# larskaislaniemi/PyLamp

Hardware: AMD Instinct MI355X
Metric: stokes_heat_mic_cell_updates_per_s (higher is better)
Workload: dtype f64

## Files before the change

include/pylamp_hip.h:

```cpp
#ifndef PYLAMP_HIP_H
#define PYLAMP_HIP_H

#include <stddef.h>
#include <stdint.h>

#ifdef __cplusplus
extern "C" {
#endif

typedef struct pl_ctx pl_ctx;

enum { PL_BC_NOSLIP = 0, PL_BC_FREESLIP = 1, PL_BC_CYCLIC = 2, PL_BC_FLOWTHRU = 4 };
enum { PL_BC_FIXTEMP = 0, PL_BC_FIXFLOW = 1 };
enum { PL_AVG_ARITHMETIC = 1, PL_AVG_GEOMETRIC = 2, PL_AVG_WEIGHTED = 4 };
enum { PL_INTERP_NEAREST = 8, PL_INTERP_LINEAR = 16, PL_INTERP_VELDIV = 32 };

typedef struct pl_solve_stats {
    int    iterations;
    int    converged;
    double rel_residual;
    double solve_ms;
    int    operator_applies;
    int    precond_applies;
    int    used_direct;
    int    reserved_;
    double error_estimate;
} pl_solve_stats;

int  pl_create(pl_ctx** out, int device, int nz, int nx, const double* zc, const double* xc);
void pl_destroy(pl_ctx* ctx);
const char* pl_last_error(const pl_ctx* ctx);
int  pl_sync(pl_ctx* ctx);
int  pl_device_info(pl_ctx* ctx, char* name, size_t name_len, int* cu_count, size_t* hbm_bytes);

typedef struct pl_comm_ops {
    int (*sendrecv)(void* user, int nmsg, const int* peer, const double* const* send, const int64_t* nsend,
                    double* const* recv, const int64_t* nrecv);
    int (*allreduce_host)(void* user, double* buf, int64_t n, int op);
    int (*allgather)(void* user, const double* send, double* recv, int64_t count);
    void* user;
} pl_comm_ops;
int  pl_set_comm(pl_ctx* ctx, int rank, int nranks, const pl_comm_ops* ops);
int  pl_set_comm_2d(pl_ctx* ctx, int rank, int Pz, int Px, const pl_comm_ops* ops);
int  pl_local_rows(pl_ctx* ctx, int* first_row, int* n_rows);
int  pl_local_block(pl_ctx* ctx, int* first_row, int* n_rows, int* first_col, int* n_cols, int* Pz, int* Px);
typedef struct pl_local_group pl_local_group;
int  pl_local_group_create(pl_local_group** out, int nranks);
void pl_local_group_destroy(pl_local_group* g);
void pl_local_group_abort(pl_local_group* g);
int  pl_set_comm_local(pl_ctx* ctx, pl_local_group* g, int rank, int Pz, int Px);
void pl_local_group_enter(pl_local_group* g);
void pl_local_group_leave(pl_local_group* g, pl_ctx* ctx);
int  pl_comm_info(pl_ctx* ctx, int* rank, int* nranks, int* native);
int  pl_comm_stats(pl_ctx* ctx, int64_t out[4], int reset);
int  pl_comm_times(pl_ctx* ctx, double out_ms[4], int reset);
int  pl_memcpy_d2h(pl_ctx* ctx, void* dst_host, const void* src_dev, size_t bytes);
int  pl_memcpy_h2d(pl_ctx* ctx, void* dst_dev, const void* src_host, size_t bytes);
int  pl_dev_add(pl_ctx* ctx, double* dst_dev, const double* src_dev, int64_t n);

int  pl_timer_start(pl_ctx* ctx);
int  pl_timer_stop_ms(pl_ctx* ctx, double* ms);

int  pl_stokes_set_coeffs(pl_ctx* ctx, const double* etas, const double* etan, const double* rho,
                          const int bc[4], int surfstab, double tstep, double theta);
int  pl_stokes_get_scaling(pl_ctx* ctx, double* kcont, double* kbond);
int  pl_stokes_apply(pl_ctx* ctx, const double* x, double* y);
int  pl_stokes_rhs(pl_ctx* ctx, double* rhs);
int  pl_stokes_residual_dd(pl_ctx* ctx, const double* rhs, const double* x, double* r);
int  pl_stokes_direct_info(pl_ctx* ctx, int* band, int* nb, double* factor_ms, double* solve_ms, int* nsolve);
int  pl_stokes_solve(pl_ctx* ctx, const double* rhs, double* x, int use_x0, double rtol,
                     int maxit, pl_solve_stats* stats);
int  pl_stokes_apply_bench(pl_ctx* ctx, int reps, double* avg_ms);
int  pl_stokes_apply_scaled_bench(pl_ctx* ctx, int reps, double* avg_ms);
int  pl_stream_triad_bench(pl_ctx* ctx, int64_t n, int reps, double* avg_ms);

int  pl_stokes_precond_apply(pl_ctx* ctx, const double* r, double* z);
int  pl_stokes_apply_reduce(pl_ctx* ctx, int mode, int rows, const double* x, const double* aux1, const double* aux2,
                            double* out, double* out2, double* sums);
int  pl_stokes_apply_probe(pl_ctx* ctx, int scaled, int mode, int rows, const double* x, const double* aux1,
                           const double* aux2, const double* add, double coef, double* out, double* out2, double* sums);
int  pl_stokes_scale_rows(pl_ctx* ctx, const double* v, double* out);
int  pl_stokes_mg_info(pl_ctx* ctx, int* nlevels, double* lmax, int max_levels);
int  pl_stokes_mg_plan(pl_ctx* ctx, int* smoother, int max_levels, int* nu, double* ratio, int* wall_ps);
int  pl_stokes_sweep_bench(pl_ctx* ctx, int reps, double* avg_ms);
int  pl_stokes_mg_precision(pl_ctx* ctx, int* nlevels, int* nlevels_fp32);
int  pl_stokes_set_mg_precision(pl_ctx* ctx, int fp32, long long min_nodes);

int  pl_heat_set_coeffs(pl_ctx* ctx, const double* zmp, const double* xmp, const double* T,
                        const double* kz, const double* kx, const double* cp, const double* rho,
                        const double* H, const int bc[4], const double bcvalue[4], double tstep);
int  pl_heat_apply(pl_ctx* ctx, const double* x, double* y);
int  pl_heat_rhs(pl_ctx* ctx, double* rhs);
int  pl_heat_solve(pl_ctx* ctx, const double* rhs, double* x, double rtol, int maxit,
                   pl_solve_stats* stats);
int  pl_heat_apply_bench(pl_ctx* ctx, int reps, double* avg_ms);
int  pl_heat_fused_launches(pl_ctx* ctx, long long* n);

int  pl_trac2grid(pl_ctx* ctx, int64_t n, const double* tr_x, const double* tr_f, int64_t ld_f,
                  int nf, const int* avgscheme, double z0, double hz, double x0, double hx,
                  double* const* out);
int  pl_trac2grid_rect(pl_ctx* ctx, int64_t n, const double* tr_x, const double* tr_f, int64_t ld_f,
                       int nf, const int* avgscheme, const double* zc, const double* xc, double* const* out);
int  pl_mic_set_search(pl_ctx* ctx, int on);
int  pl_grid2trac(pl_ctx* ctx, int64_t n, const double* tr_x, int nf, const double* const* fields,
                  int gnz, int gnx, const double* gz, const double* gx, int method, double defval,
                  int stop_on_error, double* out, int64_t ld_out, int64_t* n_outside);
int  pl_rk4(pl_ctx* ctx, int64_t n, const double* tr_x, int gnz, int gnx, const double* gz,
            const double* gx, const double* vz, const double* vx, double tstep, double* v_out,
            double* x_out);

typedef struct pl_step_config {
    int    do_heatdiff, do_subgrid_heatdiff, tdep_rho, tdep_eta;
    double etamin, etamax, tref;
    double tstep_adv_max, tstep_adv_min, tstep_dif_max, tstep_dif_min, tstep_modifier;
    int    bcstokes[4];
    int    bcheat[4];
    double bcheatvals[4];
    double stokes_rtol, heat_rtol;
    int    stokes_maxit, heat_maxit;
    double length[2];
    int    tracdens, tracdens_min;
    uint64_t inject_seed;
    int    surface_stabilization;
    double surfstab_theta, surfstab_tstep;
    int    inject_unique_ids;
    int    tracs_fence_disabled;
} pl_step_config;

typedef struct pl_step_report {
    double tstep;
    int    limiter;
    double tstep_heat, tstep_stokes;
    pl_solve_stats stokes, heat;
    double ms_props, ms_scatter, ms_stokes, ms_heat, ms_gather, ms_advect, ms_sort, ms_total;
    int64_t ntrac;
    int64_t ninjected;
    int     stokes_resolves;
    int64_t nremoved;
} pl_step_report;

int  pl_tracers_upload(pl_ctx* ctx, int64_t n, const double* tr_x, const double* tr_f);
int  pl_tracers_download(pl_ctx* ctx, int64_t n, double* tr_x, double* tr_f);
int  pl_tracers_count(pl_ctx* ctx, int64_t* n);
int  pl_tracers_census(pl_ctx* ctx, int64_t ncells, int32_t* counts, int* first_cell_row, int* n_cell_rows);
int  pl_tracers_layout(pl_ctx* ctx, int* epoch_age, int* lazy);
int  pl_step(pl_ctx* ctx, const pl_step_config* cfg, int it, pl_step_report* rep);
int  pl_resident_scatter(pl_ctx* ctx, const pl_step_config* cfg, int it);
int  pl_resident_temp_to_tracers(pl_ctx* ctx, const pl_step_config* cfg, int first, const double* newtemp, double tstep);
int  pl_resident_rk4(pl_ctx* ctx, const double* vz_pad, const double* vx_pad, double tstep, int fence, const double length[2]);
int  pl_get_field(pl_ctx* ctx, const char* name, double* out);
int  pl_get_tracer_velocity(pl_ctx* ctx, int64_t n, double* out);

typedef struct pl3_ctx pl3_ctx;
int  pl3_create(pl3_ctx** out, int device, int nz, int nx, int ny, const double* zc, const double* xc, const double* yc);
void pl3_destroy(pl3_ctx* ctx);
const char* pl3_last_error(const pl3_ctx* ctx);
int  pl3_set_comm(pl3_ctx* ctx, pl_ctx* comm, int Pz, int Px, int Py);
int  pl3_local_block(pl3_ctx* ctx, int first[3], int count[3]);
int  pl3_comm_stats(pl3_ctx* ctx, int64_t out[2], int reset);
int  pl3_stokes_set_coeffs(pl3_ctx* ctx, const double* etas, const double* etan, const double* rho, const double grav[3]);
int  pl3_stokes_set_wall_rows(pl3_ctx* ctx, int slaved);
int  pl3_stokes_set_walls(pl3_ctx* ctx, const int bc[6]);
int  pl3_stokes_set_wall_velocity(pl3_ctx* ctx, const double vel[18]);
int  pl3_stokes_get_wall_velocity(pl3_ctx* ctx, double vel[18]);
int  pl3_stokes_get_scaling(pl3_ctx* ctx, double* kcont, double* kbond);
int  pl3_stokes_apply(pl3_ctx* ctx, const double* x, double* y);
int  pl3_stokes_rhs(pl3_ctx* ctx, double* rhs);
int  pl3_stokes_rhs_scaled(pl3_ctx* ctx, double* rhs);
int  pl3_stokes_solve(pl3_ctx* ctx, const double* rhs, double* x, int use_x0, double rtol, int maxit, pl_solve_stats* stats);
int  pl3_stokes_apply_bench(pl3_ctx* ctx, int scaled, int reps, double* avg_ms);
int  pl3_stokes_mg_info(pl3_ctx* ctx, int* nlevels, double* lmax, int max_levels);
int  pl3_heat_set_coeffs(pl3_ctx* ctx, const double* zmp, const double* xmp, const double* ymp, const double* T, const double* kz,
                         const double* kx, const double* ky, const double* cp, const double* rho, const double* H, const int bc[6],
                         const double bcvalue[6], double tstep);
int  pl3_heat_apply(pl3_ctx* ctx, const double* x, double* y);
int  pl3_heat_rhs(pl3_ctx* ctx, double* rhs);
int  pl3_heat_solve(pl3_ctx* ctx, const double* rhs, double* x, double rtol, int maxit, pl_solve_stats* stats);
int  pl3_get_solution(pl3_ctx* ctx, int which, double* out);

int  pl3_trac2grid(pl3_ctx* ctx, int64_t n, const double* tr_x, const double* tr_f, int64_t ld_f, int nf, const int* avgscheme,
                   const double* zc, int nzc, const double* xc, int nxc, const double* yc, int nyc, double* const* out);
int  pl3_grid2trac(pl3_ctx* ctx, int64_t n, const double* tr_x, int nf, const double* const* fields, int gnz, int gnx, int gny,
                   const double* gz, const double* gx, const double* gy, int method, double defval, int stop_on_error, double* out,
                   int64_t ld_out, int64_t* n_outside);
int  pl3_rk4(pl3_ctx* ctx, int64_t n, const double* tr_x, int gnz, int gnx, int gny, const double* gz, const double* gx, const double* gy,
             const double* vz, const double* vx, const double* vy, double tstep, double* v_out, double* x_out);
int  pl3_mic_set_search(pl3_ctx* ctx, int on);
int  pl3_mic_get_search(pl3_ctx* ctx, int* on);
int  pl3_tracers_upload(pl3_ctx* ctx, int64_t n, const double* tr_x, const double* tr_f);
int  pl3_tracers_download(pl3_ctx* ctx, int64_t n, double* tr_x, double* tr_f);
int  pl3_tracers_count(pl3_ctx* ctx, int64_t* n);
int  pl3_tracers_census(pl3_ctx* ctx, int64_t ncell, int32_t* counts);
int  pl3_resident_props(pl3_ctx* ctx, int tdep_rho, int tdep_eta, double tref, double etamin, double etamax);
int  pl3_resident_trac2grid(pl3_ctx* ctx, int nf, const int* columns, const int* avgscheme, const double* zc, int nzc, const double* xc,
                            int nxc, const double* yc, int nyc, double* const* out);
int  pl3_resident_temp_to_tracers(pl3_ctx* ctx, int absolute, const double* field, int subgrid, double tstep);
int  pl3_resident_rk4(pl3_ctx* ctx, const double* gz, const double* gx, const double* gy, const double* vz, const double* vx,
                      const double* vy, double tstep, int fence);
int  pl3_get_tracer_velocity(pl3_ctx* ctx, int64_t n, double* out);
int  pl3_resident_refill(pl3_ctx* ctx, int tracdens, int tracdens_min, uint64_t seed, int it, int unique_ids, int64_t out[4]);
int  pl3_resident_advect(pl3_ctx* ctx, const double* gz, const double* gx, const double* gy, const double* vz, const double* vx,
                         const double* vy, double tstep, int fence, int tracdens, int tracdens_min, uint64_t seed, int it,
                         int unique_ids, int64_t out[4]);
int  pl3_resident_times(pl3_ctx* ctx, double ms[4]);

typedef struct pl3_step_config {
    int    do_heatdiff, do_subgrid_heatdiff, tdep_rho, tdep_eta;
    double etamin, etamax, tref;
    double tstep_adv_max, tstep_adv_min, tstep_dif_max, tstep_dif_min, tstep_modifier;
    int    bcheat[6];
    double bcheatvals[6];
    double stokes_rtol, heat_rtol;
    int    stokes_maxit, heat_maxit;
    int    use_grav;
    int    reserved_;
    double grav[3];
    int    tracdens, tracdens_min;
    uint64_t inject_seed;
    int    inject_unique_ids;
    int    reserved2_;
} pl3_step_config;
typedef struct pl3_step_report {
    double tstep;
    int    limiter;
    int    reserved_;
    double tstep_heat, tstep_stokes;
    pl_solve_stats stokes, heat;
    int64_t ninjected, nrefilled, nempty, mincount;
    int64_t ntrac;
    int64_t nan_rho, nan_etas;
    double ms_scatter, ms_stokes, ms_heat, ms_gather, ms_rk4, ms_sort;
    double ms_total;
} pl3_step_report;
int  pl3_resident_step(pl3_ctx* ctx, const pl3_step_config* cfg, int it, pl3_step_report* report);
int  pl3_get_field(pl3_ctx* ctx, const char* name, double* out);
int  pl3_advection_velocity(pl3_ctx* ctx, const double* vz, const double* vx, const double* vy, double* Vz, double* Vx, double* Vy);
int  pl3_transfer_stats(pl3_ctx* ctx, int64_t out[4], int reset);
int  pl3_abi_layout(size_t out[8]);

// ... 7 lines not shown
```

pylamp_amd/_lib.py:

```python
import ctypes as C
import os

import numpy as np

_HERE = os.path.dirname(os.path.abspath(__file__))
LIB_PATH = os.path.join(_HERE, "libpylamp_hip.so")

c_double_p = C.POINTER(C.c_double)
c_int_p = C.POINTER(C.c_int)


class SolveStats(C.Structure):
    _fields_ = [("iterations", C.c_int), ("converged", C.c_int), ("rel_residual", C.c_double),
                ("solve_ms", C.c_double), ("operator_applies", C.c_int), ("precond_applies", C.c_int),
                ("used_direct", C.c_int), ("reserved_", C.c_int), ("error_estimate", C.c_double)]

    def as_dict(self):
        return {k: getattr(self, k) for k, _ in self._fields_}


class StepConfig(C.Structure):
    _fields_ = [("do_heatdiff", C.c_int), ("do_subgrid_heatdiff", C.c_int), ("tdep_rho", C.c_int),
                ("tdep_eta", C.c_int), ("etamin", C.c_double), ("etamax", C.c_double), ("tref", C.c_double),
                ("tstep_adv_max", C.c_double), ("tstep_adv_min", C.c_double), ("tstep_dif_max", C.c_double),
                ("tstep_dif_min", C.c_double), ("tstep_modifier", C.c_double), ("bcstokes", C.c_int * 4),
                ("bcheat", C.c_int * 4), ("bcheatvals", C.c_double * 4), ("stokes_rtol", C.c_double),
                ("heat_rtol", C.c_double), ("stokes_maxit", C.c_int), ("heat_maxit", C.c_int),
                ("length", C.c_double * 2), ("tracdens", C.c_int), ("tracdens_min", C.c_int),
                ("inject_seed", C.c_uint64), ("surface_stabilization", C.c_int), ("surfstab_theta", C.c_double),
                ("surfstab_tstep", C.c_double), ("inject_unique_ids", C.c_int), ("tracs_fence_disabled", C.c_int)]


class StepReport(C.Structure):
    _fields_ = [("tstep", C.c_double), ("limiter", C.c_int), ("tstep_heat", C.c_double),
                ("tstep_stokes", C.c_double), ("stokes", SolveStats), ("heat", SolveStats),
                ("ms_props", C.c_double), ("ms_scatter", C.c_double), ("ms_stokes", C.c_double),
                ("ms_heat", C.c_double), ("ms_gather", C.c_double), ("ms_advect", C.c_double),
                ("ms_sort", C.c_double), ("ms_total", C.c_double), ("ntrac", C.c_int64), ("ninjected", C.c_int64),
                ("stokes_resolves", C.c_int), ("nremoved", C.c_int64)]


class Step3Config(C.Structure):
    _fields_ = [("do_heatdiff", C.c_int), ("do_subgrid_heatdiff", C.c_int), ("tdep_rho", C.c_int), ("tdep_eta", C.c_int),
                ("etamin", C.c_double), ("etamax", C.c_double), ("tref", C.c_double),
                ("tstep_adv_max", C.c_double), ("tstep_adv_min", C.c_double), ("tstep_dif_max", C.c_double),
                ("tstep_dif_min", C.c_double), ("tstep_modifier", C.c_double), ("bcheat", C.c_int * 6),
                ("bcheatvals", C.c_double * 6), ("stokes_rtol", C.c_double), ("heat_rtol", C.c_double),
                ("stokes_maxit", C.c_int), ("heat_maxit", C.c_int), ("use_grav", C.c_int), ("reserved_", C.c_int),
                ("grav", C.c_double * 3), ("tracdens", C.c_int), ("tracdens_min", C.c_int), ("inject_seed", C.c_uint64),
                ("inject_unique_ids", C.c_int), ("reserved2_", C.c_int)]


class Step3Report(C.Structure):
    _fields_ = [("tstep", C.c_double), ("limiter", C.c_int), ("reserved_", C.c_int), ("tstep_heat", C.c_double),
                ("tstep_stokes", C.c_double), ("stokes", SolveStats), ("heat", SolveStats),
                ("ninjected", C.c_int64), ("nrefilled", C.c_int64), ("nempty", C.c_int64), ("mincount", C.c_int64),
                ("ntrac", C.c_int64), ("nan_rho", C.c_int64), ("nan_etas", C.c_int64),
                ("ms_scatter", C.c_double), ("ms_stokes", C.c_double), ("ms_heat", C.c_double), ("ms_gather", C.c_double),
                ("ms_rk4", C.c_double), ("ms_sort", C.c_double), ("ms_total", C.c_double)]


SIGNATURES = {
    "pl_create": (C.c_int, [C.POINTER(C.c_void_p), C.c_int, C.c_int, C.c_int, c_double_p, c_double_p]),
    "pl_destroy": (None, [C.c_void_p]),
    "pl_last_error": (C.c_char_p, [C.c_void_p]),
    "pl_sync": (C.c_int, [C.c_void_p]),
    "pl_abi_layout": (C.c_int, [C.POINTER(C.c_size_t)]),
    "pl3_create": (C.c_int, [C.POINTER(C.c_void_p), C.c_int, C.c_int, C.c_int, C.c_int, c_double_p, c_double_p, c_double_p]),
    "pl3_destroy": (None, [C.c_void_p]),
    "pl3_set_comm": (C.c_int, [C.c_void_p, C.c_void_p, C.c_int, C.c_int, C.c_int]),
    "pl3_local_block": (C.c_int, [C.c_void_p, c_int_p, c_int_p]),
    "pl3_comm_stats": (C.c_int, [C.c_void_p, C.POINTER(C.c_int64), C.c_int]),
    "pl3_last_error": (C.c_char_p, [C.c_void_p]),
    "pl3_stokes_set_coeffs": (C.c_int, [C.c_void_p, c_double_p, c_double_p, c_double_p, c_double_p]),
    "pl3_stokes_set_wall_rows": (C.c_int, [C.c_void_p, C.c_int]),
    "pl3_stokes_set_walls": (C.c_int, [C.c_void_p, C.POINTER(C.c_int)]),
    "pl3_stokes_set_wall_velocity": (C.c_int, [C.c_void_p, c_double_p]),
    "pl3_stokes_get_wall_velocity": (C.c_int, [C.c_void_p, c_double_p]),
    "pl3_stokes_get_scaling": (C.c_int, [C.c_void_p, c_double_p, c_double_p]),
    "pl3_stokes_apply": (C.c_int, [C.c_void_p, c_double_p, c_double_p]),
    "pl3_stokes_rhs": (C.c_int, [C.c_void_p, c_double_p]),
    "pl3_stokes_rhs_scaled": (C.c_int, [C.c_void_p, c_double_p]),
    "pl3_stokes_solve": (C.c_int, [C.c_void_p, c_double_p, c_double_p, C.c_int, C.c_double, C.c_int, C.POINTER(SolveStats)]),
    "pl3_stokes_apply_bench": (C.c_int, [C.c_void_p, C.c_int, C.c_int, c_double_p]),
    "pl3_stokes_mg_info": (C.c_int, [C.c_void_p, c_int_p, c_double_p, C.c_int]),
    "pl3_heat_set_coeffs": (C.c_int, [C.c_void_p] + [c_double_p] * 10 + [c_int_p, c_double_p, C.c_double]),
    "pl3_heat_apply": (C.c_int, [C.c_void_p, c_double_p, c_double_p]),
    "pl3_heat_rhs": (C.c_int, [C.c_void_p, c_double_p]),
    "pl3_heat_solve": (C.c_int, [C.c_void_p, c_double_p, c_double_p, C.c_double, C.c_int, C.POINTER(SolveStats)]),
    "pl3_get_solution": (C.c_int, [C.c_void_p, C.c_int, c_double_p]),
    "pl3_trac2grid": (C.c_int, [C.c_void_p, C.c_int64, c_double_p, c_double_p, C.c_int64, C.c_int, c_int_p, c_double_p, C.c_int,
                                c_double_p, C.c_int, c_double_p, C.c_int, C.POINTER(c_double_p)]),
    "pl3_grid2trac": (C.c_int, [C.c_void_p, C.c_int64, c_double_p, C.c_int, C.POINTER(c_double_p), C.c_int, C.c_int, C.c_int,
                                c_double_p, c_double_p, c_double_p, C.c_int, C.c_double, C.c_int, c_double_p, C.c_int64,
                                C.POINTER(C.c_int64)]),
    "pl3_rk4": (C.c_int, [C.c_void_p, C.c_int64, c_double_p, C.c_int, C.c_int, C.c_int] + [c_double_p] * 6 +
                [C.c_double, c_double_p, c_double_p]),
    "pl3_mic_set_search": (C.c_int, [C.c_void_p, C.c_int]),
    "pl3_mic_get_search": (C.c_int, [C.c_void_p, c_int_p]),
    "pl3_tracers_upload": (C.c_int, [C.c_void_p, C.c_int64, c_double_p, c_double_p]),
    "pl3_tracers_download": (C.c_int, [C.c_void_p, C.c_int64, c_double_p, c_double_p]),
    "pl3_tracers_count": (C.c_int, [C.c_void_p, C.POINTER(C.c_int64)]),
    "pl3_tracers_census": (C.c_int, [C.c_void_p, C.c_int64, C.POINTER(C.c_int32)]),
    "pl3_resident_props": (C.c_int, [C.c_void_p, C.c_int, C.c_int, C.c_double, C.c_double, C.c_double]),
    "pl3_resident_trac2grid": (C.c_int, [C.c_void_p, C.c_int, c_int_p, c_int_p, c_double_p, C.c_int, c_double_p, C.c_int,
                                         c_double_p, C.c_int, C.POINTER(c_double_p)]),
    "pl3_resident_temp_to_tracers": (C.c_int, [C.c_void_p, C.c_int, c_double_p, C.c_int, C.c_double]),
    "pl3_resident_rk4": (C.c_int, [C.c_void_p] + [c_double_p] * 6 + [C.c_double, C.c_int]),
    "pl3_get_tracer_velocity": (C.c_int, [C.c_void_p, C.c_int64, c_double_p]),
    "pl3_resident_refill": (C.c_int, [C.c_void_p, C.c_int, C.c_int, C.c_uint64, C.c_int, C.c_int, C.POINTER(C.c_int64)]),
    "pl3_resident_advect": (C.c_int, [C.c_void_p] + [c_double_p] * 6 + [C.c_double, C.c_int, C.c_int, C.c_int, C.c_uint64, C.c_int, C.c_int,
                                      C.POINTER(C.c_int64)]),
    "pl3_resident_times": (C.c_int, [C.c_void_p, c_double_p]),
    "pl3_resident_step": (C.c_int, [C.c_void_p, C.POINTER(Step3Config), C.c_int, C.POINTER(Step3Report)]),
    "pl3_get_field": (C.c_int, [C.c_void_p, C.c_char_p, c_double_p]),
    "pl3_advection_velocity": (C.c_int, [C.c_void_p] + [c_double_p] * 6),
    "pl3_transfer_stats": (C.c_int, [C.c_void_p, C.POINTER(C.c_int64), C.c_int]),
    "pl3_abi_layout": (C.c_int, [C.POINTER(C.c_size_t)]),
    "pl_device_info": (C.c_int, [C.c_void_p, C.c_char_p, C.c_size_t, c_int_p, C.POINTER(C.c_size_t)]),
    "pl_set_comm": (C.c_int, [C.c_void_p, C.c_int, C.c_int, C.c_void_p]),
    "pl_set_comm_2d": (C.c_int, [C.c_void_p, C.c_int, C.c_int, C.c_int, C.c_void_p]),
    "pl_local_rows": (C.c_int, [C.c_void_p, c_int_p, c_int_p]),
    "pl_local_block": (C.c_int, [C.c_void_p, c_int_p, c_int_p, c_int_p, c_int_p, c_int_p, c_int_p]),
    "pl_local_group_create": (C.c_int, [C.POINTER(C.c_void_p), C.c_int]),
    "pl_local_group_destroy": (None, [C.c_void_p]),
    "pl_local_group_abort": (None, [C.c_void_p]),
    "pl_local_group_enter": (None, [C.c_void_p]),
    "pl_local_group_leave": (None, [C.c_void_p, C.c_void_p]),
    "pl_set_comm_local": (C.c_int, [C.c_void_p, C.c_void_p, C.c_int, C.c_int, C.c_int]),
    "pl_comm_info": (C.c_int, [C.c_void_p, c_int_p, c_int_p, c_int_p]),
    "pl_comm_stats": (C.c_int, [C.c_void_p, C.POINTER(C.c_int64), C.c_int]),
    "pl_comm_times": (C.c_int, [C.c_void_p, c_double_p, C.c_int]),
    "pl_memcpy_d2h": (C.c_int, [C.c_void_p, C.c_void_p, C.c_void_p, C.c_size_t]),
    "pl_memcpy_h2d": (C.c_int, [C.c_void_p, C.c_void_p, C.c_void_p, C.c_size_t]),
    "pl_dev_add": (C.c_int, [C.c_void_p, c_double_p, c_double_p, C.c_int64]),
    "pl_timer_start": (C.c_int, [C.c_void_p]),
    "pl_timer_stop_ms": (C.c_int, [C.c_void_p, c_double_p]),
    "pl_stokes_set_coeffs": (C.c_int, [C.c_void_p, c_double_p, c_double_p, c_double_p, c_int_p, C.c_int,
                                       C.c_double, C.c_double]),
    "pl_stokes_get_scaling": (C.c_int, [C.c_void_p, c_double_p, c_double_p]),
    "pl_stokes_apply": (C.c_int, [C.c_void_p, c_double_p, c_double_p]),
    "pl_stokes_rhs": (C.c_int, [C.c_void_p, c_double_p]),
    "pl_stokes_residual_dd": (C.c_int, [C.c_void_p, c_double_p, c_double_p, c_double_p]),
    "pl_stokes_direct_info": (C.c_int, [C.c_void_p, c_int_p, c_int_p, c_double_p, c_double_p, c_int_p]),
    "pl_stokes_solve": (C.c_int, [C.c_void_p, c_double_p, c_double_p, C.c_int, C.c_double, C.c_int,
                                  C.POINTER(SolveStats)]),
    "pl_stokes_apply_bench": (C.c_int, [C.c_void_p, C.c_int, c_double_p]),
    "pl_stokes_apply_scaled_bench": (C.c_int, [C.c_void_p, C.c_int, c_double_p]),
    "pl_stream_triad_bench": (C.c_int, [C.c_void_p, C.c_int64, C.c_int, c_double_p]),
    "pl_stokes_precond_apply": (C.c_int, [C.c_void_p, c_double_p, c_double_p]),
    "pl_stokes_apply_reduce": (C.c_int, [C.c_void_p, C.c_int, C.c_int] + [c_double_p] * 6),
    "pl_stokes_apply_probe": (C.c_int, [C.c_void_p, C.c_int, C.c_int, C.c_int] + [c_double_p] * 4 + [C.c_double] + [c_double_p] * 3),
    "pl_stokes_scale_rows": (C.c_int, [C.c_void_p, c_double_p, c_double_p]),
    "pl_stokes_mg_info": (C.c_int, [C.c_void_p, c_int_p, c_double_p, C.c_int]),
    "pl_stokes_mg_plan": (C.c_int, [C.c_void_p, c_int_p, C.c_int, c_int_p, c_double_p, c_int_p]),
    "pl_stokes_mg_precision": (C.c_int, [C.c_void_p, c_int_p, c_int_p]),
    "pl_stokes_set_mg_precision": (C.c_int, [C.c_void_p, C.c_int, C.c_longlong]),
    "pl_stokes_sweep_bench": (C.c_int, [C.c_void_p, C.c_int, c_double_p]),
    "pl_heat_set_coeffs": (C.c_int, [C.c_void_p] + [c_double_p] * 8 + [c_int_p, c_double_p, C.c_double]),
    "pl_heat_apply": (C.c_int, [C.c_void_p, c_double_p, c_double_p]),
    "pl_heat_rhs": (C.c_int, [C.c_void_p, c_double_p]),
    "pl_heat_solve": (C.c_int, [C.c_void_p, c_double_p, c_double_p, C.c_double, C.c_int, C.POINTER(SolveStats)]),
    "pl_heat_apply_bench": (C.c_int, [C.c_void_p, C.c_int, c_double_p]),
    "pl_heat_fused_launches": (C.c_int, [C.c_void_p, C.POINTER(C.c_longlong)]),
    "pl_trac2grid": (C.c_int, [C.c_void_p, C.c_int64, c_double_p, c_double_p, C.c_int64, C.c_int, c_int_p,
                               C.c_double, C.c_double, C.c_double, C.c_double, C.POINTER(c_double_p)]),
    "pl_trac2grid_rect": (C.c_int, [C.c_void_p, C.c_int64, c_double_p, c_double_p, C.c_int64, C.c_int, c_int_p,
                                    c_double_p, c_double_p, C.POINTER(c_double_p)]),
    "pl_mic_set_search": (C.c_int, [C.c_void_p, C.c_int]),
    "pl_grid2trac": (C.c_int, [C.c_void_p, C.c_int64, c_double_p, C.c_int, C.POINTER(c_double_p), C.c_int,
                               C.c_int, c_double_p, c_double_p, C.c_int, C.c_double, C.c_int, c_double_p,
                               C.c_int64, C.POINTER(C.c_int64)]),
    "pl_rk4": (C.c_int, [C.c_void_p, C.c_int64, c_double_p, C.c_int, C.c_int, c_double_p, c_double_p,
                         c_double_p, c_double_p, C.c_double, c_double_p, c_double_p]),
    "pl_tracers_upload": (C.c_int, [C.c_void_p, C.c_int64, c_double_p, c_double_p]),
    "pl_tracers_download": (C.c_int, [C.c_void_p, C.c_int64, c_double_p, c_double_p]),
    "pl_tracers_count": (C.c_int, [C.c_void_p, C.POINTER(C.c_int64)]),
    "pl_tracers_census": (C.c_int, [C.c_void_p, C.c_int64, C.POINTER(C.c_int32), c_int_p, c_int_p]),
    "pl_tracers_layout": (C.c_int, [C.c_void_p, c_int_p, c_int_p]),
    "pl_step": (C.c_int, [C.c_void_p, C.POINTER(StepConfig), C.c_int, C.POINTER(StepReport)]),
    "pl_resident_scatter": (C.c_int, [C.c_void_p, C.POINTER(StepConfig), C.c_int]),
    "pl_resident_temp_to_tracers": (C.c_int, [C.c_void_p, C.POINTER(StepConfig), C.c_int, c_double_p, C.c_double]),
    "pl_resident_rk4": (C.c_int, [C.c_void_p, c_double_p, c_double_p, C.c_double, C.c_int, c_double_p]),
    "pl_get_field": (C.c_int, [C.c_void_p, C.c_char_p, c_double_p]),
    "pl_get_tracer_velocity": (C.c_int, [C.c_void_p, C.c_int64, c_double_p]),
}

_lib = None


def load():
    global _lib
    if _lib is not None:
        return _lib
    if not os.path.exists(LIB_PATH):
        raise Exception("pylamp_amd: %s is missing — run `python -c 'import __graft_entry__ as g; g.build()'` "
                        "(there is no CPU fallback)" % LIB_PATH)
    try:
        import torch
    except Exception:
        pass
    lib = C.CDLL(LIB_PATH)
    for name, (res, args) in SIGNATURES.items():
        fn = getattr(lib, name)
        fn.restype = res
        fn.argtypes = args
    _lib = lib
    return lib


def dptr(a):
    return a.ctypes.data_as(c_double_p)


def f64(a):
    return np.ascontiguousarray(a, dtype=np.float64)


def check(ctx_handle, rc):
    if rc != 0:
        msg = load().pl_last_error(ctx_handle)
        raise Exception(msg.decode() if msg else "libpylamp_hip error %d" % rc)
```

pylamp_amd/csrc/pl_solver.hip:

```cpp
#include "pl_internal.h"
#include <chrono>
#include <cmath>
#include <functional>
#include <limits>

#define TB(tab, k) (tab)[(k) + PL_TOFF]

void pl_launch_heat_rhs(pl_ctx* ctx, const PlHeatOp& op, const double* Told, const double* H, double* rhs);

template <typename T>
struct PlVvOpT {
    PlGeom g;
    const T* etas; const T* etan;
    const T *rdz, *rDz, *rdx, *rDx;
    int slave_x;
    int slave_z0, slave_zL;
    T s0, sL;
    const T* szz; const T* szx;
};
typedef PlVvOpT<double> PlVvOp;
typedef PlVvOpT<float> PlVvOpF;

enum { VV_ZERO = 0, VV_INT = 1, VV_SLAVE = 2 };

// ... 1208 lines not shown
    }
    *reinterpret_cast<VF2*>(f + c) = PlVec2<TF>::make((TF)(fz[0] * fscale), (TF)(fz[1] * fscale));
    *reinterpret_cast<VF2*>(f + PLN + c) = PlVec2<TF>::make((TF)(fx[0] * fscale), (TF)(fx[1] * fscale));
    *reinterpret_cast<double2*>(z + 2 * PLN + c) = make_double2(zp[0], zp[1]);
    if (v1) {
        const double nc2 = -c2 * v1scale;
        *reinterpret_cast<VF2*>(v1 + c) = PlVec2<TF>::make((TF)((nc2 * fz[0]) * pl_rcp(dz[0])), (TF)((nc2 * fz[1]) * pl_rcp(dz[1])));
        *reinterpret_cast<VF2*>(v1 + PLN + c) = PlVec2<TF>::make((TF)((nc2 * fx[0]) * pl_rcp(dx[0])), (TF)((nc2 * fx[1]) * pl_rcp(dx[1])));
    }
}

__global__ __launch_bounds__(256) void k_close_constraints(PlStokesOp op, PlVvOp vop, const double* __restrict__ bs,
                                                           double* __restrict__ x) {
    PL_NODE_PROLOGUE(op.g)
    const long long P = op.g.plane;
    int moff; double s;
    int cls = vv_cls_z(vop, i, j, moff, s);
    if (cls == VV_ZERO) x[c] = bs[c];
    else if (cls == VV_SLAVE) x[c] = s * x[c + moff] + bs[c];
    cls = vv_cls_x(vop, i, j, moff, s);
    if (cls == VV_ZERO) x[c + P] = bs[c + P];
    else if (cls == VV_SLAVE) {
        double g0 = bs[c + P];
        if (i == 0 && op.bc_z0 != PL_BC_FREESLIP) g0 /= (-TB(op.g.rDz, 1) - TB(op.g.rdz, 0));
        if (i == op.g.nz - 2 && op.bc_zL != PL_BC_FREESLIP) g0 /= (TB(op.g.rDz, op.g.nz - 2) + TB(op.g.rdz, op.g.nz - 2));
        x[c + P] = s * x[c + moff + P] + g0;
    }
}

#define PL_HYDRO_CHUNK 64
__global__ __launch_bounds__(64) void k_hydro_chunk(PlStokesOp op, double* __restrict__ x, double* __restrict__ ctot) {
    const PlGeom& g = op.g;
    const int lj = blockIdx.x * 64 + threadIdx.x, ch = blockIdx.y;
    if (lj >= g.lnx) return;
    double* P = x + 2 * g.plane;
    const double* r = op.rho;
    const int l0 = ch * PL_HYDRO_CHUNK, l1 = min(l0 + PL_HYDRO_CHUNK, g.lnz);
    const int jn = (g.gj0 + lj + 1 < g.nx) ? 1 : 0;
    double acc = 0.0;
    for (int li = l0; li < l1; li++) {
        const int i = g.gi0 + li;
        const long long c = pl_idx(g, li, lj);
        if (i >= 1 && i <= g.nz - 2) acc += 0.5 * (r[c] + r[c + jn]) * op.gz / (2.0 * op.Kc * TB(g.rDz, i));
        P[c] = acc;
    }
    ctot[(long long)ch * g.lnx + lj] = acc;
}
__global__ __launch_bounds__(64) void k_hydro_chunk_scan(PlGeom g, int nch, double* __restrict__ ctot, double* __restrict__ coltot) {
    const int lj = blockIdx.x * 64 + threadIdx.x;
    if (lj >= g.lnx) return;
    double acc = 0.0;
    for (int ch = 0; ch < nch; ch++) { const double t = ctot[(long long)ch * g.lnx + lj]; ctot[(long long)ch * g.lnx + lj] = acc; acc += t; }
    coltot[lj] = acc;
}
__global__ __launch_bounds__(256) void k_hydro_add(PlGeom g, double* __restrict__ x, const double* __restrict__ cpre) {
    PL_NODE_PROLOGUE(g)
    (void)i; (void)j;
    x[2 * g.plane + c] += cpre[(long long)(li / PL_HYDRO_CHUNK) * g.lnx + lj];
}

__global__ __launch_bounds__(256) void k_hydrostatic_apply_shift(PlStokesOp op, double* __restrict__ x,
                                                                 const double* __restrict__ prefix, double pa) {
    PL_NODE_PROLOGUE(op.g)
    const PlGeom& g = op.g;
    double* P = x + 2 * g.plane;
    x[c] = 0.0; x[c + g.plane] = 0.0;
    P[c] = (i >= g.nz - 1 || j >= g.nx - 1) ? 0.0 : P[c] + prefix[lj] - pa;
}

struct MgLevel {
    PlGeomHost gh;
    bool dist = false;
    PlGeom win{};
    long long win_shift = 0;
    PlVvOp op{};
    double* etas = nullptr; double* etan = nullptr; bool own_visc = false;
    double *rho = nullptr, *szz = nullptr, *szx = nullptr;
    double* eig = nullptr; bool eig_valid = false;
    int eig_confirm = 0, eig_skip = 0;
    bool own_rho = false;
    double* v[3] = {nullptr, nullptr, nullptr};
    double *f = nullptr, *r = nullptr;
    double lmax = 3.0;
    bool line_z = false;
    int line_ax = 0;
    bool f32 = false;
    PlVvOpF opf{};
    float *etas_f = nullptr, *etan_f = nullptr, *tab_f = nullptr;
    float* vf[3] = {nullptr, nullptr, nullptr};
    float *ff = nullptr, *rf = nullptr;
};
template <typename T> struct LevelT;
template <> struct LevelT<double> {
    static const PlVvOp& op(const MgLevel* L) { return L->op; }
    static double** v(MgLevel* L) { return L->v; }
    static double* f(MgLevel* L) { return L->f; }
    static double* r(MgLevel* L) { return L->r; }
};
template <> struct LevelT<float> {
    static const PlVvOpF& op(const MgLevel* L) { return L->opf; }
    static float** v(MgLevel* L) { return L->vf; }
    static float* f(MgLevel* L) { return L->ff; }
    static float* r(MgLevel* L) { return L->rf; }
};

struct PlSolver {
    std::vector<MgLevel*> levels;
    int bc_key[4] = {-1, -1, -1, -1};
    int repl_start = -1;
    long long repl_max_nodes = 300000;
    double *r = nullptr, *rt = nullptr, *p = nullptr, *v = nullptr, *s = nullptr, *t = nullptr, *y = nullptr,
           *z = nullptr, *b = nullptr, *x = nullptr, *xb = nullptr, *dx = nullptr, *r0 = nullptr, *xh = nullptr,
           *bu = nullptr;
    double* scal = nullptr;
    double* hpart = nullptr;
    double* epi = nullptr;
    long long epi_blocks = 0;
    int nu_pre = 2, nu_post = 2, coarse_sweeps = 12;
    int nu0_pre = -1, nu0_post = -1;
    bool aniso_auto = true, ratio_knob = false;
    int power_its_warm = 1;
    bool nu_auto = true;
    bool use_tail = true;
    bool any_line = false;
    long long tail_knob = 0;
    long long tail_max_nodes = 33 * 33;
    int min_cells = 4;
    bool f32_enable = false; long long f32_min_nodes = 200000;
    double etol = 3e-8;
    double kappa = 1.0, sigma = 1.0;
    bool defl_enable = true;
    bool defl_persistent = false;
    bool defl_valid = false, defl_active = false;
    double *wdefl = nullptr, *udefl = nullptr;
    double defl_yAw = 0.0, defl_wvel2 = 0.0;
    double* Awdefl = nullptr;
    bool defl_lazy = false;
    double schur_scale = 1.0;
    double ref_cached = 0.0, ref_kc = 0.0; int ref_age = 0;
    long long fused_max_nodes = 1100000;
    long long tile32_min_nodes = 1000000;
    bool fused = true;
    bool fuse_first = true;
    bool l0_mixed = true;
    bool l0_mixed_now = true;
    bool deep = true;
    int tail_nu_pre = -1, tail_nu_post = -1;
    double cheb_ratio = 6.0, lmax_safety = 1.1;
    double* h[11] = {nullptr};
    double* hc3 = nullptr;
    double* hc[9] = {nullptr}; double* hc_part = nullptr; int hc_nb = 0, hc_last_its = 0;
    int napply = 0, nprec = 0;
    long long heat_fused_launches = 0;
};

static PlSolver* solver_of(pl_ctx* ctx) {
    if (!ctx->krylov) {
        PlSolver* S = new PlSolver();
        if (const char* e = getenv("PYLAMP_MG_NU")) { int a = 0, b = 0; if (sscanf(e, "%d,%d", &a, &b) == 2 && a >= 0 && b >= 0 && a + b > 0) { S->nu_pre = a; S->nu_post = b; S->nu_auto = false; } }
        if (const char* e = getenv("PYLAMP_MG_NU0")) { int a = 0, b = 0; if (sscanf(e, "%d,%d", &a, &b) == 2 && a >= 1 && b >= 1) { S->nu0_pre = a; S->nu0_post = b; S->nu_auto = false; } }
        if (const char* e = getenv("PYLAMP_MG_POWER")) { int a = atoi(e); if (a >= 1) S->power_its_warm = a; }
        if (const char* e = getenv("PYLAMP_MG_COARSE")) { int a = atoi(e); if (a > 0) S->coarse_sweeps = a; }
        if (const char* e = getenv("PYLAMP_MG_TAIL")) S->use_tail = atoi(e) != 0;
        if (const char* e = getenv("PYLAMP_MG_REPL_NODES")) { long long v = atoll(e); if (v >= 25) S->repl_max_nodes = v; }
        if (const char* e = getenv("PYLAMP_MG_TAIL_NODES")) { long long v = atoll(e); if (v >= 25 && v <= PL_TAIL_MAX_NODES) S->tail_knob = v; }
        if (const char* e = getenv("PYLAMP_MG_DEEP")) S->deep = atoi(e) != 0;
        if (const char* e = getenv("PYLAMP_DEFLATE")) S->defl_enable = atoi(e) != 0;
        if (const char* e = getenv("PYLAMP_STOKES_ETOL")) { const double v = atof(e); if (v >= 0.0) S->etol = v; }
        if (const char* e = getenv("PYLAMP_MG_FP32")) S->f32_enable = atoi(e) != 0;
        if (const char* e = getenv("PYLAMP_MG_FP32_NODES")) { long long v = atoll(e); if (v >= 1) S->f32_min_nodes = v; }
        if (const char* e = getenv("PYLAMP_L0_MIXED")) S->l0_mixed = atoi(e) != 0;
        if (const char* e = getenv("PYLAMP_MG_FUSED")) S->fused = atoi(e) != 0;
        if (const char* e = getenv("PYLAMP_MG_TS32")) { long long v = atoll(e); if (v > 0) S->tile32_min_nodes = v; }
        if (const char* e = getenv("PYLAMP_MG_FUSED_MAX")) { long long v = atoll(e); if (v > 0) S->fused_max_nodes = v; }
        if (const char* e = getenv("PYLAMP_SCHUR_SCALE")) { double v = atof(e); if (v > 0.0) S->schur_scale = v; }
        if (const char* e = getenv("PYLAMP_MG_TAIL_NU")) { int a = 0, b = 0; if (sscanf(e, "%d,%d", &a, &b) == 2 && a + b > 0) { S->tail_nu_pre = a; S->tail_nu_post = b; } }
        if (const char* e = getenv("PYLAMP_MG_RATIO")) { double v = atof(e); if (v > 1.5) { S->cheb_ratio = v; S->ratio_knob = true; } }
        if (const char* e = getenv("PYLAMP_MG_ANISO")) S->aniso_auto = atoi(e) != 0;
        if (const char* e = getenv("PYLAMP_MG_SAFETY")) { double v = atof(e); if (v >= 1.0) S->lmax_safety = v; }
        ctx->krylov = S;
    }
    return (PlSolver*)ctx->krylov;
}

static void free_levels(PlSolver* S) {
    for (MgLevel* L : S->levels) {
        if (L->own_visc) { (void)hipFree(L->etas); (void)hipFree(L->etan); }
        if (L->own_rho && L->rho) (void)hipFree(L->rho);
        for (double* q : {L->szz, L->szx, L->eig}) if (q) (void)hipFree(q);
        for (double* q : {L->v[0], L->v[1], L->v[2], L->f, L->r}) if (q) (void)hipFree(q);
        for (float* q : {L->etas_f, L->etan_f, L->tab_f, L->vf[0], L->vf[1], L->vf[2], L->ff, L->rf}) if (q) (void)hipFree(q);
        pl_geom_free(L->gh);
        delete L;
    }
    S->levels.clear();
}

void pl_solver_free(pl_ctx* ctx) {
    PlSolver* S = (PlSolver*)ctx->krylov;
    if (!S) return;
    free_levels(S);
    for (double* q : {S->r, S->rt, S->p, S->v, S->s, S->t, S->y, S->z, S->b, S->x, S->xb, S->dx, S->r0, S->xh, S->bu, S->scal, S->wdefl, S->udefl, S->Awdefl})
        if (q) (void)hipFree(q);
    for (double* q : S->h) if (q) (void)hipFree(q);
    for (double* q : S->hc) if (q) (void)hipFree(q);
    if (S->hc_part) (void)hipFree(S->hc_part);
    if (S->hc3) (void)hipFree(S->hc3);
    if (S->hpart) (void)hipHostFree(S->hpart);
    if (S->epi) (void)hipFree(S->epi);
    delete S;
    ctx->krylov = nullptr;
}

static int dmalloc0(pl_ctx* ctx, double** p, size_t bytes) {
    PL_HIP(ctx, hipMalloc((void**)p, bytes));
    PL_HIP(ctx, hipMemsetAsync(*p, 0, bytes, ctx->stream));
    return 0;
}
static int scal_alloc(pl_ctx* ctx, PlSolver* S) {
    if (S->scal) return 0;
    PL_TRY(dmalloc0(ctx, &S->scal, (PL_SCAL_N + PL_PART_N * DOT_BLOCKS) * sizeof(double)));
    PL_HIP(ctx, hipHostMalloc((void**)&S->hpart, (PL_HSCAL + PL_SCAL_N) * sizeof(double)));
    return 0;
}

__global__ void k_scalar_alpha(double* __restrict__ sc, double rho_new) { sc[SC_ALPHA] = rho_new / sc[SC_SUM_A]; sc[SC_RHO] = rho_new; }
__global__ void k_s_update_dev(long long n, double* __restrict__ y, const double* __restrict__ a, const double* __restrict__ b,
                               const double* __restrict__ sc) {
    const double alpha = sc[SC_ALPHA];
    long long k = (long long)blockIdx.x * blockDim.x + threadIdx.x;
    for (; k < n; k += (long long)gridDim.x * blockDim.x) y[k] = a[k] - alpha * b[k];
}
template <bool FIRST>
__global__ void k_xrp_update_dev(long long n, double* __restrict__ x, const double* __restrict__ y, const double* __restrict__ z,
                                 double* __restrict__ r, const double* __restrict__ s, const double* __restrict__ t,
                                 double* __restrict__ p, const double* __restrict__ v, const double* __restrict__ sc,
                                 const double* __restrict__ wd, const double* __restrict__ awd, const double* __restrict__ p0) {
    const double alpha = sc[SC_ALPHA], omega = sc[SC_OMEGA], beta = sc[SC_BETA];
    const double cw = wd ? alpha * sc[SC_CY] + omega * sc[SC_CZ] : 0.0;
    const double cz = awd ? sc[SC_CZ] : 0.0;
    long long k = (long long)blockIdx.x * blockDim.x + threadIdx.x;
    for (; k < n; k += (long long)gridDim.x * blockDim.x) {
        double xn = FIRST ? alpha * y[k] + omega * z[k] : x[k] + alpha * y[k] + omega * z[k];
        if (wd) xn += cw * wd[k];
        x[k] = xn;
        const double rn = s[k] - omega * (awd ? t[k] + cz * awd[k] : t[k]);
        r[k] = rn;
        p[k] = rn + beta * ((FIRST ? p0[k] : p[k]) - omega * v[k]);
    }
}
__global__ void k_xr_update_dev(long long n, double* __restrict__ x, const double* __restrict__ y, const double* __restrict__ z,
                                double* __restrict__ r, const double* __restrict__ s, const double* __restrict__ t,
                                const double* __restrict__ sc) {
    const double alpha = sc[SC_ALPHA], omega = sc[SC_OMEGA];
    long long k = (long long)blockIdx.x * blockDim.x + threadIdx.x;
    for (; k < n; k += (long long)gridDim.x * blockDim.x) { x[k] += alpha * y[k] + omega * z[k]; r[k] = s[k] - omega * t[k]; }
}

__global__ __launch_bounds__(1024) void k_sum_partials(int nb, const double* __restrict__ part, double* __restrict__ out,
                                                       int mode = 0, double rho_new = 0.0) {
    double s0 = 0.0, s1 = 0.0;
    const int nt = blockDim.x, nw = nt >> 6;
#pragma unroll 2
    for (int k = threadIdx.x; k < nb; k += nt) { s0 += part[2 * k]; s1 += part[2 * k + 1]; }
    __shared__ double sh[2][16];
#pragma unroll
    for (int o = 32; o > 0; o >>= 1) { s0 += __shfl_down(s0, o, 64); s1 += __shfl_down(s1, o, 64); }
    if ((threadIdx.x & 63) == 0) { sh[0][threadIdx.x >> 6] = s0; sh[1][threadIdx.x >> 6] = s1; }
    __syncthreads();
    if (threadIdx.x == 0) {
        double a0 = sh[0][0], a1 = sh[1][0];
        for (int w = 1; w < nw; w++) { a0 += sh[0][w]; a1 += sh[1][w]; }
        out[0] = a0; out[1] = a1;
        if (mode == 1) { out[SC_ALPHA] = rho_new / a0; out[SC_RHO] = rho_new; }
    }
}

static int dots(pl_ctx* ctx, PlSolver* S, const PlGeom& g, int np, const double* a, const double* b, const double* c,
                const double* d, double* out2) {
    long long rows = (long long)g.lnz * np;
    const int nb = (int)(rows < DOT_BLOCKS ? rows : DOT_BLOCKS);
    if (a && c) hipLaunchKernelGGL((k_dot2<true, true>), dim3(nb), dim3(256), 0, ctx->stream, g, np, a, b, c, d, S->scal + SC_PART);
    else if (a) hipLaunchKernelGGL((k_dot2<true, false>), dim3(nb), dim3(256), 0, ctx->stream, g, np, a, b, c, d, S->scal + SC_PART);
    else hipLaunchKernelGGL((k_dot2<false, true>), dim3(nb), dim3(256), 0, ctx->stream, g, np, a, b, c, d, S->scal + SC_PART);
    if (ctx->nranks > 1 && pl_geom_is_dist(g)) {
        hipLaunchKernelGGL(k_sum_partials, dim3(1), dim3(256), 0, ctx->stream, nb, S->scal + SC_PART, S->scal + SC_SUM_A);
        PL_TRY(pl_comm_allreduce_dev(ctx, S->scal + SC_SUM_A, 2));
        PL_HIP(ctx, hipMemcpyAsync(S->hpart, S->scal + SC_SUM_A, 2 * sizeof(double), hipMemcpyDeviceToHost, ctx->stream));
        PL_HIP(ctx, hipStreamSynchronize(ctx->stream));
        out2[0] = S->hpart[0]; out2[1] = S->hpart[1];
        return 0;
    }
    PL_HIP(ctx, hipMemcpyAsync(S->hpart, S->scal + SC_PART, (size_t)2 * nb * sizeof(double), hipMemcpyDeviceToHost, ctx->stream));
    PL_HIP(ctx, hipStreamSynchronize(ctx->stream));
    double s0 = 0.0, s1 = 0.0;
    for (int k = 0; k < nb; k++) { s0 += S->hpart[2 * k]; s1 += S->hpart[2 * k + 1]; }
    out2[0] = s0; out2[1] = s1;
    return 0;
}

static int dots5_dev(pl_ctx* ctx, PlSolver* S, const PlGeom& g, int np, int nsplit, const double* t, const double* sv, const double* rt,
                     const double* aw_ride = nullptr) {
    long long rows = (long long)g.lnz * np;
    const int nb = (int)(rows < DOT_BLOCKS ? rows : DOT_BLOCKS);
    hipLaunchKernelGGL(k_dot5, dim3(nb), dim3(256), 0, ctx->stream, g, np, nsplit, t, sv, rt, S->scal + SC_PART);
    const bool reduce = ctx->nranks > 1 && pl_geom_is_dist(g);
// ... 294 lines not shown
                PL_TRY(pl_gather_blocks(ctx, L->gh.d, L->rho, 1, L->gh.d.plane));
            } else {
                hipLaunchKernelGGL(k_coarsen_node, grid2d(L->gh.d), dim3(64, 4), 0, ctx->stream, F->gh.d, F->rho, L->gh.d, L->rho);
            }
        }
        for (size_t l = 0; l < S->levels.size(); l++) {
            MgLevel* L = S->levels[l];
            if (L->dist) PL_TRY(pl_halo(ctx, L->gh.d, L->rho, 1, L->gh.d.plane, 2));
            hipLaunchKernelGGL(k_stab_coeffs, grid2d(L->gh.d), dim3(64, 4), 0, ctx->stream, L->op, L->rho, coef, L->szz, L->szx);
            if (L->dist) {
                const int dep = std::min(PL_RING, std::min(L->gh.d.lnz, L->gh.d.lnx));
                PL_TRY(pl_halo(ctx, L->gh.d, L->szz, 1, L->gh.d.plane, dep));
                PL_TRY(pl_halo(ctx, L->gh.d, L->szx, 1, L->gh.d.plane, dep));
            }
            L->op.szz = L->szz; L->op.szx = L->szx;
        }
    }
    PL_HIP(ctx, hipGetLastError());
    for (MgLevel* L : S->levels) {
        const PlGeom& g = L->gh.d;
        long long n2 = 2 * g.plane;
        if (!L->eig) { PL_TRY(dmalloc0(ctx, &L->eig, (size_t)n2 * sizeof(double))); L->eig_valid = false; }
        if (S->defl_persistent && L->eig_valid && L->eig_confirm >= 2 && L->eig_skip < 3 && L->lmax > 0.0) { L->eig_skip++; continue; }
        L->eig_skip = 0;
        const double lam_before = (L->eig_valid && S->lmax_safety > 0.0) ? L->lmax / S->lmax_safety : 0.0;
        if (L->eig_valid) PL_HIP(ctx, hipMemcpyAsync(L->v[0], L->eig, (size_t)n2 * sizeof(double), hipMemcpyDeviceToDevice, ctx->stream));
        else hipLaunchKernelGGL(k_random_interior, grid2d(g), dim3(64, 4), 0, ctx->stream, g, 2, L->v[0], 777u);
        const bool warm = L->eig_valid;
        double lam = (warm && L->lmax > 0.0 && S->lmax_safety > 0.0) ? L->lmax / S->lmax_safety : 2.5, lam_prev = 0.0, nn[2];
        for (int it = 0; it < 12; it++) {
            if (warm && it >= S->power_its_warm && std::fabs(lam - lam_prev) < 0.01 * lam) break;
            lam_prev = lam;
            if (L->dist) PL_TRY(pl_halo(ctx, g, L->v[0], 2, g.plane));
            if (L->line_z) PL_TRY(line_z_launch(ctx, L->op, L->v[0], nullptr, nullptr, L->v[1], 0.0, 1.0, 1.0, 1, L->line_ax));
            else hipLaunchKernelGGL(k_vv_dinv_apply, grid2d(g), dim3(64, 4), 0, ctx->stream, L->op, L->v[0], L->v[1]);
            PL_TRY(dots(ctx, S, g, 2, L->v[1], L->v[1], L->v[0], L->v[0], nn));
            if (!(nn[1] > 0.0) || !(nn[0] > 0.0)) break;
            lam = std::sqrt(nn[0] / nn[1]);
            hipLaunchKernelGGL(k_axpy_out, grid1d(n2), dim3(256), 0, ctx->stream, n2, L->v[0], L->v[1], L->v[1],
                               1.0 / std::sqrt(nn[0]) - 1.0);
        }
        L->lmax = S->lmax_safety * lam;
        PL_HIP(ctx, hipMemcpyAsync(L->eig, L->v[0], (size_t)n2 * sizeof(double), hipMemcpyDeviceToDevice, ctx->stream));
        L->eig_valid = std::isfinite(lam) && lam > 0.0;
        L->eig_confirm = (L->eig_valid && lam_before > 0.0 && std::fabs(lam - lam_before) < 0.002 * lam) ? L->eig_confirm + 1 : 0;
    }
    PL_TRY(setup_f32_levels(ctx, S));
    return 0;
}

static const bool g_vv_vec_env = [] { const char* e = getenv("PYLAMP_VV_VEC"); return !(e && e[0] == '0'); }();
#define g_vv_vec (g_vv_vec_env && !(L->gh.d.gj0 & 1))

template <typename T> struct ExtViewT { PlVvOpT<T> op; long long sh; };
template <typename T>
static ExtViewT<T> ext_view(pl_ctx* ctx, const MgLevel* L, int e) {
    ExtViewT<T> v; v.op = LevelT<T>::op(L); v.sh = 0;
    if (e <= 0 || !L->dist) return v;
    const PlGeom& g = L->gh.d;
    const int a = ctx->pz > 0 ? e : 0, b = ctx->pz < ctx->Pz - 1 ? e : 0;
    const int c = ctx->px > 0 ? ((e + 1) & ~1) : 0, d = ctx->px < ctx->Px - 1 ? e : 0;
    v.op.g.gi0 -= a; v.op.g.lnz += a + b; v.op.g.gj0 -= c; v.op.g.lnx += c + d;
    v.sh = (long long)a * g.pitch + c;
    v.op.etas -= v.sh; v.op.etan -= v.sh;
    if (v.op.szz) { v.op.szz -= v.sh; v.op.szx -= v.sh; }
    return v;
}
template <typename T>
static bool smooth(pl_ctx* ctx, MgLevel* L, T* buf[3], const T* f, int nsweep, double ratio,
                   double* final_out = nullptr, double final_scale = 1.0, bool zero_guess = false,
                   bool first_halo_valid = false, int ext_first = -1, const int* first_done_anchor = nullptr) {
    const double lmax = L->lmax, lmin = lmax / ratio;
    const double theta = 0.5 * (lmax + lmin), delta = 0.5 * (lmax - lmin), sigma = theta / delta;
    double rho_old = 1.0 / sigma;
    bool wrote_final = false;
    for (int k = 0; k < nsweep; k++) {
        double c1, c2;
        if (k == 0) { c1 = 0.0; c2 = 1.0 / theta; }
        else { const double rho = 1.0 / (2.0 * sigma - rho_old); c1 = rho * rho_old; c2 = 2.0 * rho / delta; rho_old = rho; }
        if (ext_first < 0 && L->dist && !(k == 0 && (zero_guess || first_halo_valid)))
            (void)pl_halo(ctx, L->gh.d, buf[0], 2, L->gh.d.plane);
        const ExtViewT<T> V = ext_view<T>(ctx, L, ext_first < 0 ? 0 : std::max(ext_first - k, 0));
        const long long sh = V.sh;
        const bool to_final = final_out && k == nsweep - 1;
        T* dst = buf[2];
        if constexpr (std::is_same<T, double>::value) {
            if (L->line_z) {
                const double* cur = (k == 0 && zero_guess) ? nullptr : buf[0];
                const double* prv = (k == 0 || (k == 1 && zero_guess)) ? nullptr : buf[1];
                (void)line_z_launch(ctx, L->op, cur, prv, f, to_final ? final_out : dst, c1, c2, to_final ? final_scale : 1.0, 0, L->line_ax);
                if (to_final) { wrote_final = true; break; }
                { T* nxt = buf[2]; buf[2] = buf[1]; buf[1] = buf[0]; buf[0] = nxt; }
                continue;
            }
        }
        if (k == 0 && zero_guess) {
            if (g_vv_vec && first_done_anchor) {
                const dim3 full = pl_grid_rows2(V.op.g);
                hipLaunchKernelGGL(k_vv_first2<T>, dim3(3 * full.x + 3 * full.y + 2), dim3(64, 4), 0, ctx->stream, V.op, f - sh, dst - sh, (T)c2, 2,
                                   first_done_anchor[0], first_done_anchor[1], ctx->sop.wall_ps);
            }
            else if (g_vv_vec) hipLaunchKernelGGL(k_vv_first2<T>, pl_grid_rows2(V.op.g), dim3(64, 4), 0, ctx->stream, V.op, f - sh, dst - sh, (T)c2, 0, -9, -9, 0);
            else hipLaunchKernelGGL(k_vv_cheb_first<T>, pl_grid_rows(V.op.g), dim3(64, 4), 0, ctx->stream, V.op, f - sh, dst - sh, (T)c2,
                                    pl_row_iters(V.op.g));
        } else {
            const T* prev = (k == 1 && zero_guess) ? (const T*)nullptr : buf[1] - sh;
            if (to_final) {
                if (g_vv_vec)
                    hipLaunchKernelGGL((k_vv_sweep2<0, T, double>), pl_grid_rows2(V.op.g), dim3(64, 4), 0, ctx->stream, V.op, (const T*)(buf[0] - sh), prev,
                                       f - sh, final_out - sh, (T)c1, (T)c2, final_scale);
                else
                    hipLaunchKernelGGL((k_vv_cheb<T, double>), pl_grid_rows(V.op.g), dim3(64, 4), 0, ctx->stream, V.op, (const T*)(buf[0] - sh), prev, f - sh,
                                       final_out - sh, (T)c1, (T)c2, pl_row_iters(V.op.g), final_scale);
                wrote_final = true;
                break;
            }
            if (g_vv_vec)
                hipLaunchKernelGGL((k_vv_sweep2<0, T, T>), pl_grid_rows2(V.op.g), dim3(64, 4), 0, ctx->stream, V.op, (const T*)(buf[0] - sh), prev,
                                   f - sh, dst - sh, (T)c1, (T)c2, T(1));
            else
                hipLaunchKernelGGL((k_vv_cheb<T, T>), pl_grid_rows(V.op.g), dim3(64, 4), 0, ctx->stream, V.op, (const T*)(buf[0] - sh), prev, f - sh,
                                   dst - sh, (T)c1, (T)c2, pl_row_iters(V.op.g), T(1));
        }
        { T* nxt = buf[2]; buf[2] = buf[1]; buf[1] = buf[0]; buf[0] = nxt; }
    }
    return wrote_final;
}

static int coarsest_sweeps(const PlSolver* S, const PlGeom& g) {
    double ratio = 0.4 * g.nz * g.nx; if (ratio < 30.0) ratio = 30.0;
    int n = (int)std::sqrt(ratio);
    if (n < S->coarse_sweeps) n = S->coarse_sweeps;
    if (n > 150) n = 150;
    return n;
}

static void level_nu(const PlSolver* S, size_t l, int& npre, int& npost) {
    npre = (l == 0 && S->nu0_pre > 0) ? S->nu0_pre : S->nu_pre;
    npost = (l == 0 && S->nu0_post > 0) ? S->nu0_post : S->nu_post;
}
static bool level_deep_plan(const PlSolver* S, const MgLevel* L, size_t l, int& e_last, int& f_depth) {
    int npre, npost;
    level_nu(S, l, npre, npost);
    e_last = std::max(2, npost);
    f_depth = e_last + std::max(npre, 1) - 1;
    if (!L->dist || !S->deep || l + 1 == S->levels.size() || npre < 1) return false;
    return f_depth <= PL_RING - 1 && f_depth + 1 <= std::min(L->gh.d.lnz, L->gh.d.lnx);
}

template <typename T> static void vcycle(pl_ctx* ctx, PlSolver* S, size_t l, const T* f, T** out, bool* wrote_final, double* final_out,
                                         double final_scale, int f_valid_depth, const int* first_done_anchor);
static bool mg_fused_level_ok(pl_ctx* ctx, const PlSolver* S, size_t l);
static bool mg_tail_lds_fits(const PlSolver* S, size_t l);
__global__ void k_mg_tail_lds(TailArgs a);
static void vcycle_fused_level(pl_ctx* ctx, PlSolver* S, size_t l, const double* f, double** out, double* final_out, double final_scale,
                               const PlStokesOp* sop, const double* rs, double* z);

template <typename T, typename TC>
static void coarse_correction(pl_ctx* ctx, PlSolver* S, size_t l, MgLevel* L, MgLevel* C, T* buf[3], bool deep, int npost) {
    const PlGeom& g = L->gh.d;
    T* r = LevelT<T>::r(L);
    TC* cf = LevelT<TC>::f(C);
    const TC cscale = (std::is_same<T, float>::value && std::is_same<TC, double>::value) ? (TC)S->sigma : TC(1);
    if (L->dist && !C->dist) {
        PlVvOpT<TC> wop = LevelT<TC>::op(C); wop.g = C->win;
        const long long sh = C->win_shift;
        hipLaunchKernelGGL((k_vv_restrict<T, TC>), grid2d(C->win), dim3(64, 4), 0, ctx->stream, g, wop, (const T*)r, cf + sh, cscale);
        if constexpr (std::is_same<TC, double>::value) (void)pl_gather_blocks(ctx, C->gh.d, cf, 2, C->gh.d.plane);
    } else {
        hipLaunchKernelGGL((k_vv_restrict<T, TC>), grid2d(C->gh.d), dim3(64, 4), 0, ctx->stream, g, LevelT<TC>::op(C), (const T*)r, cf, cscale);
    }
    TC* ec = nullptr;
    bool wf = false;
    vcycle<TC>(ctx, S, l + 1, cf, &ec, &wf, nullptr, 1.0, 0, nullptr);
    const int pe = deep ? npost : (L->dist ? 1 : 0);
    if (C->dist)
        (void)pl_halo(ctx, C->gh.d, ec, 2, C->gh.d.plane, std::min(std::max((pe + 1) / 2 + 1, 2), std::min(PL_RING, std::min(C->gh.d.lnz, C->gh.d.lnx))));
    ExtViewT<T> V = ext_view<T>(ctx, L, pe);
    if (!deep && pe == 1) {
        V.op = LevelT<T>::op(L);
        const int lo = ctx->pz > 0 ? 1 : 0, hi = ctx->pz < ctx->Pz - 1 ? 1 : 0, we = ctx->px > 0 ? 1 : 0, ea = ctx->px < ctx->Px - 1 ? 1 : 0;
        V.op.g.gi0 -= lo; V.op.g.lnz += lo + hi; V.op.g.gj0 -= we; V.op.g.lnx += we + ea;
        V.sh = (long long)lo * g.pitch + we;
    }
    hipLaunchKernelGGL((k_vv_prolong_add<T, TC>), grid2d(V.op.g), dim3(64, 4), 0, ctx->stream, V.op, C->gh.d, (const TC*)ec, (const T*)(buf[0] - V.sh),
                       buf[2] - V.sh);
}

template <typename T>
static void vcycle(pl_ctx* ctx, PlSolver* S, size_t l, const T* f, T** out, bool* wrote_final, double* final_out,
                   double final_scale, int f_valid_depth, const int* first_done_anchor) {
    MgLevel* L = S->levels[l];
    const PlGeom& g = L->gh.d;
    *wrote_final = false;
    if constexpr (std::is_same<T, double>::value) {
        if (S->use_tail && !S->any_line && l > 0 && (long long)g.nz * g.nx <= S->tail_max_nodes &&
            S->levels.size() - l <= PL_TAIL_MAX_LEVELS && f == L->f) {
            TailArgs ta{};
            ta.nlev = (int)(S->levels.size() - l);
            ta.nu_pre = S->tail_nu_pre >= 0 ? S->tail_nu_pre : S->nu_pre; ta.nu_post = S->tail_nu_post >= 0 ? S->tail_nu_post : S->nu_post;
            ta.coarse_sweeps = coarsest_sweeps(S, S->levels.back()->gh.d); ta.ratio = S->cheb_ratio;
            for (int q = 0; q < ta.nlev; q++) {
                MgLevel* T_ = S->levels[l + q];
                ta.L[q].op = T_->op; ta.L[q].f = T_->f; ta.L[q].r = T_->r; ta.L[q].lmax = T_->lmax;
                for (int b = 0; b < 3; b++) ta.L[q].v[b] = T_->v[b];
            }
            if (S->fused && !L->dist && !L->op.szz && ta.nu_pre >= 1 && ta.nu_post >= 1 && ta.coarse_sweeps >= 1 && mg_tail_lds_fits(S, l))
                hipLaunchKernelGGL(k_mg_tail_lds, dim3(1), dim3(1024), 0, ctx->stream, ta);
            else
                hipLaunchKernelGGL(k_mg_tail, dim3(1), dim3(1024), 0, ctx->stream, ta);
            *out = L->v[0];
            return;
        }
    }
    if constexpr (std::is_same<T, double>::value) {
        if (l > 0 && !final_out && f == L->f && mg_fused_level_ok(ctx, S, l)) {
            vcycle_fused_level(ctx, S, l, f, out, nullptr, 1.0, nullptr, nullptr, nullptr);
            return;
        }
    }
    T** lv = LevelT<T>::v(L);
    T* buf[3] = {lv[0], lv[1], lv[2]};
    const bool coarsest = l + 1 == S->levels.size();
    if (!coarsest && S->nu_pre == 0)
        (void)hipMemsetAsync(buf[0], 0, (size_t)2 * g.plane * sizeof(T), ctx->stream);
    if (coarsest) {
        double ratio = 0.4 * g.nz * g.nx; if (ratio < 30.0) ratio = 30.0;
        smooth<T>(ctx, L, buf, f, coarsest_sweeps(S, g), ratio, nullptr, 1.0, true);
        *out = buf[0];
        return;
    }
    int npre, npost, e_last, f_depth;
    level_nu(S, l, npre, npost);
    const bool deep = level_deep_plan(S, L, l, e_last, f_depth);
    MgLevel* C = S->levels[l + 1];
    T* r = LevelT<T>::r(L);
    if (deep) {
        if (f_valid_depth < f_depth) (void)pl_halo(ctx, g, (T*)f, 2, g.plane, f_depth);
        smooth<T>(ctx, L, buf, f, npre, S->cheb_ratio, nullptr, 1.0, true, false, e_last + npre - 1, first_done_anchor);
        const ExtViewT<T> V = ext_view<T>(ctx, L, e_last - 1);
        if (g_vv_vec)
            hipLaunchKernelGGL((k_vv_sweep2<1, T, T>), pl_grid_rows2(V.op.g), dim3(64, 4), 0, ctx->stream, V.op, (const T*)(buf[0] - V.sh),
                               (const T*)nullptr, f - V.sh, r - V.sh, T(0), T(0), T(1));
        else
            hipLaunchKernelGGL(k_vv_residual<T>, pl_grid_rows(V.op.g), dim3(64, 4), 0, ctx->stream, V.op, (const T*)(buf[0] - V.sh), f - V.sh,
                               r - V.sh, pl_row_iters(V.op.g));
    } else {
        smooth<T>(ctx, L, buf, f, npre, S->cheb_ratio, nullptr, 1.0, true, false, -1, first_done_anchor);
        if (L->dist) (void)pl_halo(ctx, g, buf[0], 2, g.plane);
        if (g_vv_vec)
            hipLaunchKernelGGL((k_vv_sweep2<1, T, T>), pl_grid_rows2(g), dim3(64, 4), 0, ctx->stream, LevelT<T>::op(L), (const T*)buf[0], (const T*)nullptr, f,
                               r, T(0), T(0), T(1));
        else
            hipLaunchKernelGGL(k_vv_residual<T>, pl_grid_rows(g), dim3(64, 4), 0, ctx->stream, LevelT<T>::op(L), (const T*)buf[0], f, r, pl_row_iters(g));
        if (L->dist) (void)pl_halo(ctx, g, r, 2, g.plane, 2);
    }
    if constexpr (std::is_same<T, float>::value) {
        if (C->f32) coarse_correction<float, float>(ctx, S, l, L, C, buf, deep, npost);
        else coarse_correction<float, double>(ctx, S, l, L, C, buf, deep, npost);
    } else {
        coarse_correction<double, double>(ctx, S, l, L, C, buf, deep, npost);
    }
    std::swap(buf[0], buf[2]);
    if (deep) *wrote_final = smooth<T>(ctx, L, buf, f, npost, S->cheb_ratio, final_out, final_scale, false, true, npost - 1);
    else *wrote_final = smooth<T>(ctx, L, buf, f, npost, S->cheb_ratio, final_out, final_scale, false, L->dist);
    *out = buf[0];
}

#define MGT_TS 16
#ifndef MGT_NT
#define MGT_NT 1024
#endif
struct MgTileArgs {
    PlVvOp op;
    PlVvOp opc;
    const double* f; double* fout;
    double* v;
    double* fc;
    const double* ec;
    double* out; double oscale; long long out_plane;
    double c1[4], c2[4];
    PlStokesOp sop; const double* rs; double* z;
    int tiles_x;
};

struct MgtTab { const double* es; const double* en; const double* rdz; const double* rDz; const double* rdx; const double* rDx; };

__device__ inline int mgt_cls_z(const PlVvOp& op, int i, int j, int& db, double& s) {
    db = 0; s = 1.0;
    if (i <= 0 || i >= op.g.nz - 1 || j < 0 || j >= op.g.nx - 1) return VV_ZERO;
    if (op.slave_x) {
        if (j == 0) { db = 1; return VV_SLAVE; }
        if (j == op.g.nx - 2) { db = -1; return VV_SLAVE; }
    }
    return VV_INT;
}
__device__ inline int mgt_cls_x(const PlVvOp& op, int i, int j, int& da, double& s) {
    da = 0; s = 1.0;
    if (j <= 0 || j >= op.g.nx - 1 || i < 0 || i >= op.g.nz - 1) return VV_ZERO;
    if (i == 0 && op.slave_z0) { da = 1; s = op.s0; return VV_SLAVE; }
    if (i == op.g.nz - 2 && op.slave_zL) { da = -1; s = op.sL; return VV_SLAVE; }
    return VV_INT;
}
template <bool NEED_A>
__device__ inline void mgt_row_z(const MgtTab& t, const int CR, const double* vz, const double* vx, int c, int a, int b, double& Av, double& dg) {
    const double rdz_i = t.rdz[a + 1], rdz_m = t.rdz[a], rDz_i = t.rDz[a + 1];
    const double rdx_j = t.rdx[b + 1], rDx_j = t.rDx[b + 1], rDx_p = t.rDx[b + 2];
    const double esC = t.es[c], esE = t.es[c + 1];
    const double cN = 4.0 * t.en[c] * rdz_i * rDz_i, cS = 4.0 * t.en[c - CR] * rdz_m * rDz_i;
    const double cE = 2.0 * esE * rDx_p * rdx_j, cW = 2.0 * esC * rDx_j * rdx_j;
    dg = cN + cS + cE + cW;
    if (NEED_A) {
        const double xE = 2.0 * esE * rDz_i * rdx_j, xW = 2.0 * esC * rDz_i * rdx_j;
        const double v0 = vz[c];
        Av = cN * (vz[c + CR] - v0) - cS * (v0 - vz[c - CR]) + cE * (vz[c + 1] - v0) - cW * (v0 - vz[c - 1]) +
             xE * (vx[c + 1] - vx[c - CR + 1]) - xW * (vx[c] - vx[c - CR]);
    }
}
template <bool NEED_A>
__device__ inline void mgt_row_x(const MgtTab& t, const int CR, const double* vz, const double* vx, int c, int a, int b, double& Av, double& dg) {
    const double rdx_j = t.rdx[b + 1], rdx_m = t.rdx[b], rDx_j = t.rDx[b + 1];
    const double rdz_i = t.rdz[a + 1], rDz_i = t.rDz[a + 1], rDz_p = t.rDz[a + 2];
    const double esC = t.es[c], esN = t.es[c + CR];
    const double cE = 4.0 * t.en[c] * rdx_j * rDx_j, cW = 4.0 * t.en[c - 1] * rdx_m * rDx_j;
    const double cN = 2.0 * esN * rDz_p * rdz_i, cS = 2.0 * esC * rDz_i * rdz_i;
    dg = cE + cW + cN + cS;
    if (NEED_A) {
        const double zN = 2.0 * esN * rDx_j * rdz_i, zS = 2.0 * esC * rDx_j * rdz_i;
        const double v0 = vx[c];
        Av = cE * (vx[c + 1] - v0) - cW * (v0 - vx[c - 1]) + cN * (vx[c + CR] - v0) - cS * (v0 - vx[c - CR]) +
             zN * (vz[c + CR] - vz[c + CR - 1]) - zS * (vz[c] - vz[c - 1]);
    }
}

struct MgtTile {
    int ci0, cj0;
    int CR, NR;
    MgtTab t;
    __device__ inline void first(const PlVvOp& op, const double* fz, const double* fx, double* oz, double* ox, double c2, int a, int b) const {
        const int i = ci0 + a, j = cj0 + b, c = a * CR + b;
        int d; double s, Av, dg;
        double o = 0.0;
        int cls = mgt_cls_z(op, i, j, d, s);
        if (cls != VV_ZERO && b + d >= 1 && b + d <= CR - 2) { mgt_row_z<false>(t, CR, nullptr, nullptr, c + d, a, b + d, Av, dg); o = (-s * c2 * fz[c + d]) * pl_rcp(dg); }
        oz[c] = o;
        o = 0.0;
        cls = mgt_cls_x(op, i, j, d, s);
        if (cls != VV_ZERO && a + d >= 1 && a + d <= NR - 2) { mgt_row_x<false>(t, CR, nullptr, nullptr, c + d * CR, a + d, b, Av, dg); o = (-s * c2 * fx[c + d * CR]) * pl_rcp(dg); }
        ox[c] = o;
    }
    __device__ inline void cheb(const PlVvOp& op, const double* vz, const double* vx, const double* pz, const double* px, const double* fz,
                                const double* fx, double c1, double c2, int a, int b, double& oz, double& ox) const {
        const int i = ci0 + a, j = cj0 + b, c = a * CR + b;
        int d; double s, Av, dg;
        oz = 0.0; ox = 0.0;
        int cls = mgt_cls_z(op, i, j, d, s);
        if (cls != VV_ZERO && b + d >= 1 && b + d <= CR - 2) {
            const int cm = c + d;
            mgt_row_z<true>(t, CR, vz, vx, cm, a, b + d, Av, dg);
            const double v0 = vz[cm], mom = (c1 != 0.0) ? c1 * (v0 - (pz ? pz[cm] : 0.0)) : 0.0;
            oz = s * (v0 + mom + (c2 * (Av - fz[cm])) * pl_rcp(dg));
        }
        cls = mgt_cls_x(op, i, j, d, s);
        if (cls != VV_ZERO && a + d >= 1 && a + d <= NR - 2) {
            const int cm = c + d * CR;
            mgt_row_x<true>(t, CR, vz, vx, cm, a + d, b, Av, dg);
            const double v0 = vx[cm], mom = (c1 != 0.0) ? c1 * (v0 - (px ? px[cm] : 0.0)) : 0.0;
            ox = s * (v0 + mom + (c2 * (Av - fx[cm])) * pl_rcp(dg));
        }
    }
};

__device__ inline void mgt_load_table(double* dst, const double* tab, int first_global, int count, int n) {
    for (int k = threadIdx.x; k < count; k += blockDim.x) {
        const int gk = first_global + k;
        dst[k] = (gk >= -PL_TOFF && gk < n + PL_TOFF) ? TB(tab, gk) : 0.0;
    }
}

struct MgtC { double c0, c1, c2, c3, x0, x1, rdg, s, f; int cm, d; bool on, interior; };
template <bool ZC>
__device__ inline MgtC mgt_classify(const PlVvOp& op, int CR, int NR, int ci0, int cj0, int a, int b) {
    MgtC k; k.c0 = k.c1 = k.c2 = k.c3 = k.x0 = k.x1 = k.rdg = k.f = 0.0; k.s = 1.0; k.cm = a * CR + b; k.d = 0; k.on = false; k.interior = false;
    if (a < 1 || a > NR - 2 || b < 1 || b > CR - 2) return k;
    int d; double s;
    const int cls = ZC ? mgt_cls_z(op, ci0 + a, cj0 + b, d, s) : mgt_cls_x(op, ci0 + a, cj0 + b, d, s);
    const int am = ZC ? a : a + d, bm = ZC ? b + d : b;
    if (cls == VV_ZERO || am < 1 || am > NR - 2 || bm < 1 || bm > CR - 2) return k;
    k.s = s; k.cm = am * CR + bm; k.d = d; k.on = true; k.interior = cls == VV_INT;
    return k;
}
template <bool ZC>
__device__ inline void mgt_coefficients(MgtC& k, const MgtTab& t, int CR) {
    if (!k.on) return;
    const int c = k.cm, am = c / CR, bm = c - am * CR;
    if (ZC) {
        const double rdz_i = t.rdz[am + 1], rdz_m = t.rdz[am], rDz_i = t.rDz[am + 1];
        const double rdx_j = t.rdx[bm + 1], rDx_j = t.rDx[bm + 1], rDx_p = t.rDx[bm + 2];
        const double esC = t.es[c], esE = t.es[c + 1];
        k.c0 = 4.0 * t.en[c] * rdz_i * rDz_i; k.c1 = 4.0 * t.en[c - CR] * rdz_m * rDz_i;
        k.c2 = 2.0 * esE * rDx_p * rdx_j; k.c3 = 2.0 * esC * rDx_j * rdx_j;
        k.x0 = 2.0 * esE * rDz_i * rdx_j; k.x1 = 2.0 * esC * rDz_i * rdx_j;
    } else {
        const double rdx_j = t.rdx[bm + 1], rdx_m = t.rdx[bm], rDx_j = t.rDx[bm + 1];
        const double rdz_i = t.rdz[am + 1], rDz_i = t.rDz[am + 1], rDz_p = t.rDz[am + 2];
        const double esC = t.es[c], esN = t.es[c + CR];
        k.c0 = 4.0 * t.en[c] * rdx_j * rDx_j; k.c1 = 4.0 * t.en[c - 1] * rdx_m * rDx_j;
        k.c2 = 2.0 * esN * rDz_p * rdz_i; k.c3 = 2.0 * esC * rDz_i * rdz_i;
        k.x0 = 2.0 * esN * rDx_j * rdz_i; k.x1 = 2.0 * esC * rDx_j * rdz_i;
    }
    k.rdg = pl_rcp(k.c0 + k.c1 + k.c2 + k.c3);
}
__device__ inline double mgt_dg(const MgtC& k) { return k.c0 + k.c1 + k.c2 + k.c3; }
__device__ inline double mgt_av_z(const MgtC& k, int CR, const double* vz, const double* vx, double& v0) {
    const int c = k.cm; v0 = vz[c];
    return k.c0 * (vz[c + CR] - v0) - k.c1 * (v0 - vz[c - CR]) + k.c2 * (vz[c + 1] - v0) - k.c3 * (v0 - vz[c - 1]) +
           k.x0 * (vx[c + 1] - vx[c - CR + 1]) - k.x1 * (vx[c] - vx[c - CR]);
}
__device__ inline double mgt_av_x(const MgtC& k, int CR, const double* vz, const double* vx, double& v0) {
    const int c = k.cm; v0 = vx[c];
    return k.c0 * (vx[c + 1] - v0) - k.c1 * (v0 - vx[c - 1]) + k.c2 * (vx[c + CR] - v0) - k.c3 * (v0 - vx[c - CR]) +
           k.x0 * (vz[c + CR] - vz[c + CR - 1]) - k.x1 * (vz[c] - vz[c - 1]);
}
__device__ inline void mgt_cheb(const MgtC& kz, const MgtC& kx, int CR, const double* vz, const double* vx, double& pvz, double& pvx,
                                double c1, double c2, double& oz, double& ox) {
    oz = 0.0; ox = 0.0;
    if (kz.on) {
        double v0; const double Av = mgt_av_z(kz, CR, vz, vx, v0);
        const double mom = (c1 != 0.0) ? c1 * (v0 - pvz) : 0.0;
        oz = kz.s * (v0 + mom + (c2 * (Av - kz.f)) * kz.rdg);
        pvz = v0;
    }
    if (kx.on) {
        double v0; const double Av = mgt_av_x(kx, CR, vz, vx, v0);
        const double mom = (c1 != 0.0) ? c1 * (v0 - pvx) : 0.0;
        ox = kx.s * (v0 + mom + (c2 * (Av - kx.f)) * kx.rdg);
        pvx = v0;
    }
}
__device__ inline bool mgt_owns(int ra, int rb, int HC, int TS, int i, int j, const PlGeom& g) {
    return ra >= HC && (ra < HC + TS || (ra == HC + TS && i == g.nz - 1)) && rb >= HC && (rb < HC + TS || (rb == HC + TS && j == g.nx - 1));
}
__host__ __device__ constexpr int mgt_npt(int nn) { return (nn + 1023) / 1024; }
__host__ __device__ constexpr int mgt_nt(int nn) { return ((nn + mgt_npt(nn) - 1) / mgt_npt(nn) + 63) / 64 * 64; }
__host__ __device__ constexpr int mgt_pre_nn(int NS, int TS) { return (TS + 2 * (NS + 2)) * (TS + 2 * (NS + 2)); }
__host__ __device__ constexpr int mgt_post_nn(int NS, int TS) { return (TS + 2 * (NS + 1)) * (TS + 2 * (NS + 1)); }

template <int NS, bool L0, int TS, int EXT = 0>
__global__ __launch_bounds__(mgt_nt(mgt_pre_nn(NS + EXT, TS))) void k_mg_pre(MgTileArgs a) {
    constexpr int H = NS + 1 + EXT, HC = H + 1, CR = TS + 2 * HC, NN = CR * CR, NPT = mgt_npt(NN), NT = mgt_nt(NN);
    __shared__ double V[2][2][NN];
    __shared__ double ZP[L0 ? NN : 1];
    __shared__ double TAB[4][CR + 4];
    double* const ES = V[1][0]; double* const EN = V[1][1];
    const PlGeom& g = a.op.g;
    const int tid = threadIdx.x;
    const int ty = blockIdx.x / a.tiles_x, tx = blockIdx.x % a.tiles_x;
    const int ti0 = g.gi0 + ty * TS, tj0 = g.gj0 + tx * TS;
    const int ci0 = ti0 - HC, cj0 = tj0 - HC;
    MgtTab t; t.es = ES; t.en = EN; t.rdz = TAB[0]; t.rDz = TAB[1]; t.rdx = TAB[2]; t.rDx = TAB[3];
    mgt_load_table(TAB[0], a.op.rdz, ci0 - 1, CR + 3, g.nz); mgt_load_table(TAB[1], a.op.rDz, ci0 - 1, CR + 3, g.nz);
    mgt_load_table(TAB[2], a.op.rdx, cj0 - 1, CR + 3, g.nx); mgt_load_table(TAB[3], a.op.rDx, cj0 - 1, CR + 3, g.nx);
    const long long P = g.plane;
    MgtC kz[NPT], kx[NPT];
    int depth[NPT];
#pragma unroll
    for (int q = 0; q < NPT; q++) {
        const int idx = tid + q * NT;
        const bool have = idx < NN;
        const int ra = have ? idx / CR : 0, rb = have ? idx % CR : 0, i = ci0 + ra, j = cj0 + rb;
        depth[q] = have ? min(min(ra, CR - 1 - ra), min(rb, CR - 1 - rb)) : -1;
        kz[q] = mgt_classify<true>(a.op, CR, CR, ci0, cj0, ra, rb);
        kx[q] = mgt_classify<false>(a.op, CR, CR, ci0, cj0, ra, rb);
        const bool inmem = i - g.gi0 >= -PL_RING && i - g.gi0 < g.lnz + PL_RING && j - g.gj0 >= -PL_RING && j - g.gj0 < g.lnx + PL_RING;
        const long long c = pl_idx(g, i - g.gi0, j - g.gj0);
        const double* const fsrc = L0 ? a.rs : a.f;
        if (kz[q].on) kz[q].f = fsrc[c + kz[q].d];
        if (kx[q].on) kx[q].f = fsrc[c + (long long)kx[q].d * g.pitch + P];
        if (have) {
            ES[idx] = inmem ? a.op.etas[c] : 0.0; EN[idx] = inmem ? a.op.etan[c] : 0.0;
            if (L0) {
                const bool indom = i >= 0 && i < g.nz && j >= 0 && j < g.nx;
                ZP[idx] = indom ? prec_p_value(a.sop, a.rs + 2 * P, i, j, c) : 0.0;
            }
        }
    }
    __syncthreads();
#pragma unroll
    for (int q = 0; q < NPT; q++) {
        mgt_coefficients<true>(kz[q], t, CR); mgt_coefficients<false>(kx[q], t, CR);
        if (L0) {
            const int idx = tid + q * NT;
            const int ra = depth[q] >= 0 ? idx / CR : 0, rb = depth[q] >= 0 ? idx % CR : 0, i = ci0 + ra, j = cj0 + rb;
            if (kz[q].on) kz[q].f = kz[q].f * mgt_dg(kz[q]) + 2.0 * a.sop.Kc * TAB[1][ra + 1] * (ZP[kz[q].cm] - ZP[kz[q].cm - CR]);
            if (kx[q].on) kx[q].f = kx[q].f * mgt_dg(kx[q]) + 2.0 * a.sop.Kc * TAB[3][rb + 1] * (ZP[kx[q].cm] - ZP[kx[q].cm - 1]);
            if (depth[q] >= 0 && mgt_owns(ra, rb, HC, TS, i, j, g) && i < g.nz && j < g.nx && i - g.gi0 < g.lnz && j - g.gj0 < g.lnx) {
                const long long c = pl_idx(g, i - g.gi0, j - g.gj0);
                a.fout[c] = kz[q].interior ? kz[q].f : 0.0; a.fout[c + P] = kx[q].interior ? kx[q].f : 0.0; a.z[c + 2 * P] = ZP[idx];
            }
        }
    }
    int cur = 0;
#pragma unroll
    for (int q = 0; q < NPT; q++) {
        const int idx = tid + q * NT;
        if (depth[q] >= HC - H) {
            V[0][0][idx] = kz[q].on ? (-kz[q].s * a.c2[0] * kz[q].f) * kz[q].rdg : 0.0;
            V[0][1][idx] = kx[q].on ? (-kx[q].s * a.c2[0] * kx[q].f) * kx[q].rdg : 0.0;
        }
    }
    __syncthreads();
    double pvz[NPT], pvx[NPT];
#pragma unroll
    for (int q = 0; q < NPT; q++) { pvz[q] = 0.0; pvx[q] = 0.0; }
#pragma unroll
    for (int k = 1; k < NS; k++) {
        const int h = H - k;
#pragma unroll
        for (int q = 0; q < NPT; q++) {
            const int idx = tid + q * NT;
            if (depth[q] >= HC - h) {
                double oz, ox;
                mgt_cheb(kz[q], kx[q], CR, V[cur][0], V[cur][1], pvz[q], pvx[q], a.c1[k], a.c2[k], oz, ox);
                V[cur ^ 1][0][idx] = oz; V[cur ^ 1][1][idx] = ox;
            }
// ... 11 lines not shown
            if (kx[q].interior) rx = kx[q].f - mgt_av_x(kx[q], CR, V[cur][0], V[cur][1], v0);
            V[nxt][0][idx] = rz; V[nxt][1][idx] = rx;
        }
        if (depth[q] >= HC - (EXT ? NS : 1)) {
            const int ra = idx / CR, rb = idx % CR, i = ci0 + ra, j = cj0 + rb, li = i - g.gi0, lj = j - g.gj0;
            const bool owned = li >= 0 && li < g.lnz && lj >= 0 && lj < g.lnx;
            const bool ring = EXT && !owned && li >= -NS && li < g.lnz + NS && lj >= -NS && lj < g.lnx + NS;
            if (i >= 0 && i < g.nz && j >= 0 && j < g.nx && ((owned && mgt_owns(ra, rb, HC, TS, i, j, g)) || ring)) {
                const long long c = pl_idx(g, li, lj);
                a.v[c] = V[cur][0][idx]; a.v[c + P] = V[cur][1][idx];
            }
        }
    }
    __syncthreads();
    const PlGeom& gc = a.opc.g;
    for (int idx = tid; idx < (TS / 2 + 1) * (TS / 2 + 1); idx += NT) {
        const int u_ = idx / (TS / 2 + 1), w_ = idx % (TS / 2 + 1);
        const int I = (ti0 >> 1) + u_, J = (tj0 >> 1) + w_;
        if ((u_ == TS / 2 && I != gc.nz - 1) || (w_ == TS / 2 && J != gc.nx - 1)) continue;
        if (I >= gc.nz || J >= gc.nx || 2 * I - g.gi0 >= g.lnz || 2 * J - g.gj0 >= g.lnx) continue;
        const int b0 = (2 * I - ci0) * CR + (2 * J - cj0);
        int d; double s;
        double oz = 0.0, ox = 0.0;
        if (vv_cls_z(a.opc, I, J, d, s) == VV_INT) {
            const double wz[3] = {0.25, 0.5, 0.25}, wx[4] = {0.125, 0.375, 0.375, 0.125};
#pragma unroll
            for (int u = 0; u < 3; u++)
#pragma unroll
                for (int w = 0; w < 4; w++) oz += wz[u] * wx[w] * V[nxt][0][b0 + (u - 1) * CR + (w - 1)];
        }
        if (vv_cls_x(a.opc, I, J, d, s) == VV_INT) {
            const double wz[4] = {0.125, 0.375, 0.375, 0.125}, wx[3] = {0.25, 0.5, 0.25};
#pragma unroll
            for (int u = 0; u < 4; u++)
#pragma unroll
                for (int w = 0; w < 3; w++) ox += wz[u] * wx[w] * V[nxt][1][b0 + (u - 1) * CR + (w - 1)];
        }
        const long long cc = pl_idx(gc, I - gc.gi0, J - gc.gj0);
        a.fc[cc] = oz; a.fc[cc + gc.plane] = ox;
    }
}

template <int NS, int TS>
__global__ __launch_bounds__(mgt_nt(mgt_post_nn(NS, TS))) void k_mg_post(MgTileArgs a) {
    constexpr int H = NS, HC = H + 1, CR = TS + 2 * HC, NN = CR * CR, ECR = TS / 2 + H + 6, ENN = ECR * ECR, NPT = mgt_npt(NN), NT = mgt_nt(NN);
    __shared__ double V[2][2][NN];
    __shared__ double EC[2][ENN];
    __shared__ double TAB[4][CR + 4];
    double* const ES = V[0][0]; double* const EN = V[0][1];
    const PlGeom& g = a.op.g; const PlGeom& gc = a.opc.g;
    const int tid = threadIdx.x;
    const int ty = blockIdx.x / a.tiles_x, tx = blockIdx.x % a.tiles_x;
    const int ti0 = g.gi0 + ty * TS, tj0 = g.gj0 + tx * TS;
    const int ci0 = ti0 - HC, cj0 = tj0 - HC;
    MgtTab t; t.es = ES; t.en = EN; t.rdz = TAB[0]; t.rDz = TAB[1]; t.rdx = TAB[2]; t.rDx = TAB[3];
    mgt_load_table(TAB[0], a.op.rdz, ci0 - 1, CR + 3, g.nz); mgt_load_table(TAB[1], a.op.rDz, ci0 - 1, CR + 3, g.nz);
    mgt_load_table(TAB[2], a.op.rdx, cj0 - 1, CR + 3, g.nx); mgt_load_table(TAB[3], a.op.rDx, cj0 - 1, CR + 3, g.nx);
    const long long P = g.plane;
    const int eI0 = ((ti0 - H) >> 1) - 2, eJ0 = ((tj0 - H) >> 1) - 2;
    MgtC kz[NPT], kx[NPT];
    int depth[NPT];
#pragma unroll
    for (int q = 0; q < NPT; q++) {
        const int idx = tid + q * NT;
        const bool have = idx < NN;
        const int ra = have ? idx / CR : 0, rb = have ? idx % CR : 0, i = ci0 + ra, j = cj0 + rb;
        depth[q] = have ? min(min(ra, CR - 1 - ra), min(rb, CR - 1 - rb)) : -1;
        kz[q] = mgt_classify<true>(a.op, CR, CR, ci0, cj0, ra, rb);
        kx[q] = mgt_classify<false>(a.op, CR, CR, ci0, cj0, ra, rb);
        const bool inmem = i - g.gi0 >= -PL_RING && i - g.gi0 < g.lnz + PL_RING && j - g.gj0 >= -PL_RING && j - g.gj0 < g.lnx + PL_RING;
        const long long c = pl_idx(g, i - g.gi0, j - g.gj0);
        if (kz[q].on) kz[q].f = a.f[c + kz[q].d];
        if (kx[q].on) kx[q].f = a.f[c + (long long)kx[q].d * g.pitch + P];
        if (have) {
            ES[idx] = inmem ? a.op.etas[c] : 0.0; EN[idx] = inmem ? a.op.etan[c] : 0.0;
            V[1][0][idx] = inmem ? a.v[c] : 0.0; V[1][1][idx] = inmem ? a.v[c + P] : 0.0;
        }
    }
    for (int idx = tid; idx < ENN; idx += NT) {
        const int I = eI0 + idx / ECR, J = eJ0 + idx % ECR;
        const bool inmem = I - gc.gi0 >= -PL_RING && I - gc.gi0 < gc.lnz + PL_RING && J - gc.gj0 >= -PL_RING && J - gc.gj0 < gc.lnx + PL_RING;
        const long long cc = pl_idx(gc, I - gc.gi0, J - gc.gj0);
        EC[0][idx] = inmem ? a.ec[cc] : 0.0; EC[1][idx] = inmem ? a.ec[cc + gc.plane] : 0.0;
    }
    __syncthreads();
#pragma unroll
    for (int q = 0; q < NPT; q++) { mgt_coefficients<true>(kz[q], t, CR); mgt_coefficients<false>(kx[q], t, CR); }
    __syncthreads();
    auto ecz = [&](int I, int J) { return EC[0][(I - eI0) * ECR + (J - eJ0)]; };
    auto ecx = [&](int I, int J) { return EC[1][(I - eI0) * ECR + (J - eJ0)]; };
#pragma unroll
    for (int q = 0; q < NPT; q++) {
        const int idx = tid + q * NT;
        if (depth[q] >= HC - H) {
            const int ra = idx / CR, rb = idx % CR, i = ci0 + ra, j = cj0 + rb;
            int d; double s;
            double oz = 0.0, ox = 0.0;
            if (mgt_cls_z(a.op, i, j, d, s) != VV_ZERO) {
                const int jm = j + d;
                const int I0 = i >> 1, I1 = (i + 1) >> 1;
                int Jn = jm >> 1, Jo = (jm & 1) ? Jn + 1 : Jn - 1;
                Jn = min(max(Jn, 0), gc.nx - 2); Jo = min(max(Jo, 0), gc.nx - 2);
                const double pa = 0.5 * (ecz(I0, Jn) + ecz(I1, Jn)), pb = 0.5 * (ecz(I0, Jo) + ecz(I1, Jo));
                oz = s * (V[1][0][idx + d] + (0.75 * pa + 0.25 * pb));
            }
            if (mgt_cls_x(a.op, i, j, d, s) != VV_ZERO) {
                const int im = i + d;
                const int J0 = j >> 1, J1 = (j + 1) >> 1;
                int In = im >> 1, Io = (im & 1) ? In + 1 : In - 1;
                In = min(max(In, 0), gc.nz - 2); Io = min(max(Io, 0), gc.nz - 2);
                const double pa = 0.5 * (ecx(In, J0) + ecx(In, J1)), pb = 0.5 * (ecx(Io, J0) + ecx(Io, J1));
                ox = s * (V[1][1][idx + d * CR] + (0.75 * pa + 0.25 * pb));
            }
            V[0][0][idx] = oz; V[0][1][idx] = ox;
        }
    }
    __syncthreads();
    int cur = 0;
    double pvz[NPT], pvx[NPT];
#pragma unroll
    for (int q = 0; q < NPT; q++) { pvz[q] = 0.0; pvx[q] = 0.0; }
#pragma unroll
    for (int k = 0; k < NS; k++) {
        const int h = H - 1 - k;
#pragma unroll
        for (int q = 0; q < NPT; q++) {
            const int idx = tid + q * NT;
            if (depth[q] >= HC - h) {
                double oz, ox;
                mgt_cheb(kz[q], kx[q], CR, V[cur][0], V[cur][1], pvz[q], pvx[q], k == 0 ? 0.0 : a.c1[k], a.c2[k], oz, ox);
                if (k == NS - 1) {
                    const int ra = idx / CR, rb = idx % CR, i = ci0 + ra, j = cj0 + rb;
                    if (i < g.nz && j < g.nx && i - g.gi0 < g.lnz && j - g.gj0 < g.lnx) {
                        const long long c = pl_idx(g, i - g.gi0, j - g.gj0); a.out[c] = oz * a.oscale; a.out[c + a.out_plane] = ox * a.oscale;
                    }
                } else { V[cur ^ 1][0][idx] = oz; V[cur ^ 1][1][idx] = ox; }
            }
        }
        if (k < NS - 1) { __syncthreads(); cur ^= 1; }
    }
#pragma unroll
    for (int q = 0; q < NPT; q++) {
        const int idx = tid + q * NT;
        if (depth[q] == HC - 1) {
            const int ra = idx / CR, rb = idx % CR, i = ci0 + ra, j = cj0 + rb;
            if (mgt_owns(ra, rb, HC, TS, i, j, g) && i - g.gi0 < g.lnz && j - g.gj0 < g.lnx) {
                const long long c = pl_idx(g, i - g.gi0, j - g.gj0); a.out[c] = 0.0; a.out[c + a.out_plane] = 0.0;
            }
        }
    }
}

#define MGT_TAIL_POOL 18600
struct TailLvl { int base, NR, CR, N; };
#define TL_V(D, buf, c) (pool + (D).base + (2 * (buf) + (c)) * (D).N)
#define TL_F(D, c) (pool + (D).base + (6 + (c)) * (D).N)
#define TL_ES(D) (pool + (D).base + 8 * (D).N)
#define TL_EN(D) (pool + (D).base + 9 * (D).N)
#define TL_TAB(D, k) (pool + (D).base + 10 * (D).N + ((k) < 2 ? (k) * ((D).NR + 3) : 2 * ((D).NR + 3) + ((k) - 2) * ((D).CR + 3)))
#define TL_FOR_NODES(g)                                                                                                     \
    for (int idx = threadIdx.x, nxm_ = (g).nx - 1, pw_ = (nxm_ & (nxm_ - 1)) == 0, sh_ = 31 - __clz(nxm_), i, j;            \
         idx < ((g).nz - 1) * nxm_ && (i = pw_ ? idx >> sh_ : idx / nxm_, j = idx - i * nxm_, true); idx += MGT_NT)
__device__ inline MgtTile mgt_tail_tile(double* pool, const TailLvl& D) {
    MgtTile T; T.ci0 = -1; T.cj0 = -1; T.CR = D.CR; T.NR = D.NR;
    T.t.es = TL_ES(D); T.t.en = TL_EN(D); T.t.rdz = TL_TAB(D, 0); T.t.rDz = TL_TAB(D, 1); T.t.rdx = TL_TAB(D, 2); T.t.rDx = TL_TAB(D, 3);
    return T;
}
__device__ inline void mgt_tail_smooth(double* pool, const TailLevel& L, const TailLvl& D, int& cur, int& prv, int& nxt, int nsweep, double ratio, bool zero_guess) {
    const double lmax = L.lmax, lmin = lmax / ratio;
    const double theta = 0.5 * (lmax + lmin), delta = 0.5 * (lmax - lmin), sigma = theta / delta;
    double rho_old = 1.0 / sigma;
    const MgtTile T = mgt_tail_tile(pool, D);
    for (int k = 0; k < nsweep; k++) {
        double c1, c2;
        if (k == 0) { c1 = 0.0; c2 = 1.0 / theta; }
        else { const double rho = 1.0 / (2.0 * sigma - rho_old); c1 = rho * rho_old; c2 = 2.0 * rho / delta; rho_old = rho; }
        double* const nz_ = TL_V(D, nxt, 0); double* const nx_ = TL_V(D, nxt, 1);
        const double* const cz = TL_V(D, cur, 0); const double* const cx = TL_V(D, cur, 1);
        const bool noprev = k == 1 && zero_guess;
        const double* const pz = noprev ? nullptr : TL_V(D, prv, 0); const double* const px = noprev ? nullptr : TL_V(D, prv, 1);
        TL_FOR_NODES(L.op.g) {
            const int ra = i + 1, rb = j + 1;
            if (k == 0 && zero_guess) T.first(L.op, TL_F(D, 0), TL_F(D, 1), nz_, nx_, c2, ra, rb);
            else {
                double oz, ox;
                T.cheb(L.op, cz, cx, pz, px, TL_F(D, 0), TL_F(D, 1), c1, c2, ra, rb, oz, ox);
                nz_[ra * D.CR + rb] = oz; nx_[ra * D.CR + rb] = ox;
            }
        }
        __syncthreads();
        const int o = prv; prv = cur; cur = nxt; nxt = o;
    }
}
__global__ __launch_bounds__(MGT_NT) void k_mg_tail_lds(TailArgs a) {
    __shared__ double pool[MGT_TAIL_POOL];
    __shared__ TailLvl lv[PL_TAIL_MAX_LEVELS];
    __shared__ int rot[PL_TAIL_MAX_LEVELS];
    const int tid = threadIdx.x;
    for (int k = tid; k < MGT_TAIL_POOL; k += MGT_NT) pool[k] = 0.0;
    if (tid == 0) {
        int q = 0;
        for (int l = 0; l < a.nlev; l++) {
            const PlGeom& g = a.L[l].op.g;
            TailLvl D; D.base = q; D.NR = g.nz + 2; D.CR = g.nx + 2; D.N = D.NR * D.CR;
            q += 10 * D.N + 2 * (D.NR + 3) + 2 * (D.CR + 3);
            lv[l] = D;
        }
    }
    __syncthreads();
    for (int l = 0; l < a.nlev; l++) {
        const TailLevel& L = a.L[l]; const PlGeom& g = L.op.g; const TailLvl D = lv[l];
        for (int idx = tid; idx < g.nz * g.nx; idx += MGT_NT) {
            const int i = idx / g.nx, j = idx - i * g.nx;
            const long long c = pl_idx(g, i - g.gi0, j - g.gj0);
            const int o = (i + 1) * D.CR + (j + 1);
            TL_ES(D)[o] = L.op.etas[c]; TL_EN(D)[o] = L.op.etan[c];
            if (l == 0) { TL_F(D, 0)[o] = L.f[c]; TL_F(D, 1)[o] = L.f[c + g.plane]; }
        }
        mgt_load_table(TL_TAB(D, 0), L.op.rdz, -2, D.NR + 3, g.nz); mgt_load_table(TL_TAB(D, 1), L.op.rDz, -2, D.NR + 3, g.nz);
        mgt_load_table(TL_TAB(D, 2), L.op.rdx, -2, D.CR + 3, g.nx); mgt_load_table(TL_TAB(D, 3), L.op.rDx, -2, D.CR + 3, g.nx);
    }
    __syncthreads();
    for (int l = 0; l < a.nlev; l++) {
        const TailLevel& L = a.L[l]; const PlGeom& g = L.op.g; const TailLvl D = lv[l];
        int cur = 0, prv = 1, nxt = 2;
        if (l == a.nlev - 1) {
            double ratio = 0.4 * g.nz * g.nx; if (ratio < 30.0) ratio = 30.0;
            mgt_tail_smooth(pool, L, D, cur, prv, nxt, a.coarse_sweeps, ratio, true);
            if (tid == 0) rot[l] = cur | (prv << 2) | (nxt << 4);
            break;
        }
        mgt_tail_smooth(pool, L, D, cur, prv, nxt, a.nu_pre, a.ratio, true);
        if (tid == 0) rot[l] = cur | (prv << 2) | (nxt << 4);
        const MgtTile T = mgt_tail_tile(pool, D);
        double* const rz = TL_V(D, nxt, 0); double* const rx = TL_V(D, nxt, 1);
        const double* const cz = TL_V(D, cur, 0); const double* const cx = TL_V(D, cur, 1);
        TL_FOR_NODES(g) {
            const int ra = i + 1, rb = j + 1, o = ra * D.CR + rb;
            int d; double s, Av, dg, vz = 0.0, vx = 0.0;
            if (mgt_cls_z(L.op, i, j, d, s) == VV_INT) { mgt_row_z<true>(T.t, D.CR, cz, cx, o, ra, rb, Av, dg); vz = TL_F(D, 0)[o] - Av; }
            if (mgt_cls_x(L.op, i, j, d, s) == VV_INT) { mgt_row_x<true>(T.t, D.CR, cz, cx, o, ra, rb, Av, dg); vx = TL_F(D, 1)[o] - Av; }
            rz[o] = vz; rx[o] = vx;
        }
        __syncthreads();
        const TailLevel& Cn = a.L[l + 1]; const TailLvl Dc = lv[l + 1];
        double* const fz = TL_F(Dc, 0); double* const fx = TL_F(Dc, 1);
        TL_FOR_NODES(Cn.op.g) {
            const int b0 = (2 * i + 1) * D.CR + (2 * j + 1);
            int d; double s, oz = 0.0, ox = 0.0;
            if (vv_cls_z(Cn.op, i, j, d, s) == VV_INT) {
                const double wz[3] = {0.25, 0.5, 0.25}, wx[4] = {0.125, 0.375, 0.375, 0.125};
#pragma unroll
                for (int u = 0; u < 3; u++)
#pragma unroll
                    for (int w = 0; w < 4; w++) oz += wz[u] * wx[w] * rz[b0 + (u - 1) * D.CR + (w - 1)];
            }
            if (vv_cls_x(Cn.op, i, j, d, s) == VV_INT) {
                const double wz[4] = {0.125, 0.375, 0.375, 0.125}, wx[3] = {0.25, 0.5, 0.25};
#pragma unroll
                for (int u = 0; u < 4; u++)
#pragma unroll
                    for (int w = 0; w < 3; w++) ox += wz[u] * wx[w] * rx[b0 + (u - 1) * D.CR + (w - 1)];
            }
            const int oc = (i + 1) * Dc.CR + (j + 1);
            fz[oc] = oz; fx[oc] = ox;
        }
        __syncthreads();
    }
    __syncthreads();
    for (int l = a.nlev - 2; l >= 0; l--) {
        const TailLevel& L = a.L[l]; const PlGeom& g = L.op.g; const TailLvl D = lv[l];
        const PlGeom& gc = a.L[l + 1].op.g; const TailLvl Dc = lv[l + 1];
        int cur = rot[l] & 3, prv = (rot[l] >> 2) & 3, nxt = (rot[l] >> 4) & 3;
        const int curc = rot[l + 1] & 3;
        const double* const ez = TL_V(Dc, curc, 0); const double* const ex = TL_V(Dc, curc, 1);
        const double* const cz = TL_V(D, cur, 0); const double* const cx = TL_V(D, cur, 1);
        double* const wz_ = TL_V(D, nxt, 0); double* const wx_ = TL_V(D, nxt, 1);
        TL_FOR_NODES(g) {
            const int o = (i + 1) * D.CR + (j + 1);
            int d; double s, oz = 0.0, ox = 0.0;
            if (mgt_cls_z(L.op, i, j, d, s) != VV_ZERO) {
                const int jm = j + d, I0 = i >> 1, I1 = (i + 1) >> 1;
                int Jn = jm >> 1, Jo = (jm & 1) ? Jn + 1 : Jn - 1;
                Jn = min(max(Jn, 0), gc.nx - 2); Jo = min(max(Jo, 0), gc.nx - 2);
                const double pa = 0.5 * (ez[(I0 + 1) * Dc.CR + Jn + 1] + ez[(I1 + 1) * Dc.CR + Jn + 1]);
                const double pb = 0.5 * (ez[(I0 + 1) * Dc.CR + Jo + 1] + ez[(I1 + 1) * Dc.CR + Jo + 1]);
                oz = s * (cz[o + d] + (0.75 * pa + 0.25 * pb));
            }
            if (mgt_cls_x(L.op, i, j, d, s) != VV_ZERO) {
                const int im = i + d, J0 = j >> 1, J1 = (j + 1) >> 1;
                int In = im >> 1, Io = (im & 1) ? In + 1 : In - 1;
                In = min(max(In, 0), gc.nz - 2); Io = min(max(Io, 0), gc.nz - 2);
                const double pa = 0.5 * (ex[(In + 1) * Dc.CR + J0 + 1] + ex[(In + 1) * Dc.CR + J1 + 1]);
                const double pb = 0.5 * (ex[(Io + 1) * Dc.CR + J0 + 1] + ex[(Io + 1) * Dc.CR + J1 + 1]);
                ox = s * (cx[o + d * D.CR] + (0.75 * pa + 0.25 * pb));
            }
            wz_[o] = oz; wx_[o] = ox;
        }
        __syncthreads();
        { const int o = cur; cur = nxt; nxt = o; }
        mgt_tail_smooth(pool, L, D, cur, prv, nxt, a.nu_post, a.ratio, false);
        if (tid == 0) rot[l] = cur | (prv << 2) | (nxt << 4);
        __syncthreads();
    }
    {
        const TailLevel& L = a.L[0]; const PlGeom& g = L.op.g; const TailLvl D = lv[0];
        const int cur = rot[0] & 3;
        const double* const cz = TL_V(D, cur, 0); const double* const cx = TL_V(D, cur, 1);
        for (int idx = tid; idx < g.nz * g.nx; idx += MGT_NT) {
            const int i = idx / g.nx, j = idx - i * g.nx, o = (i + 1) * D.CR + (j + 1);
            const long long c = pl_idx(g, i - g.gi0, j - g.gj0);
            L.v[0][c] = cz[o]; L.v[0][c + g.plane] = cx[o];
        }
    }
}
static bool mg_tail_lds_fits(const PlSolver* S, size_t l) {
    long long need = 0;
    for (size_t q = l; q < S->levels.size(); q++) {
        const PlGeom& g = S->levels[q]->gh.d;
        need += 10LL * (g.nz + 2) * (g.nx + 2) + 2LL * (g.nz + 5) + 2LL * (g.nx + 5);
    }
    return need <= MGT_TAIL_POOL;
}

static void cheb_coeffs(double lmax, double ratio, int n, double* c1, double* c2) {
    const double lmin = lmax / ratio, theta = 0.5 * (lmax + lmin), delta = 0.5 * (lmax - lmin), sigma = theta / delta;
    double rho_old = 1.0 / sigma;
    for (int k = 0; k < n; k++) {
        if (k == 0) { c1[k] = 0.0; c2[k] = 1.0 / theta; }
        else { const double rho = 1.0 / (2.0 * sigma - rho_old); c1[k] = rho * rho_old; c2[k] = 2.0 * rho / delta; rho_old = rho; }
    }
}
static bool mg_fused_level_ok(pl_ctx* ctx, const PlSolver* S, size_t l) {
    if (!S->fused || l + 1 >= S->levels.size() || S->any_line) return false;
    const MgLevel* L = S->levels[l];
    if (L->f32 || L->op.szz) return false;
    const PlGeom& g = L->gh.d;
    int npre_, npost_;
    level_nu(S, l, npre_, npost_);
    if (L->dist) {
        const bool dist_fused = !(getenv("PYLAMP_MG_FUSED_DIST") && atoi(getenv("PYLAMP_MG_FUSED_DIST")) == 0);
        const MgLevel* C = S->levels[l + 1];
        if (!dist_fused || l == 0 || npre_ + 2 > std::min(g.lnz, g.lnx) || npre_ + 3 > PL_RING) return false;
        if (C->dist && std::min(C->gh.d.lnz, C->gh.d.lnx) < 4) return false;
        if ((g.gi0 & 1) || (g.gj0 & 1)) return false;
    } else if (S->levels[l + 1]->dist) return false;
    if ((long long)g.lnz * g.lnx > S->fused_max_nodes) return false;
    if (S->use_tail && l > 0 && (long long)g.nz * g.nx <= S->tail_max_nodes && S->levels.size() - l <= PL_TAIL_MAX_LEVELS) return false;
    int npre, npost;
    level_nu(S, l, npre, npost);
    return npre >= 1 && npre <= 3 && npost >= 1 && npost <= 3;
}
static void vcycle_fused_level(pl_ctx* ctx, PlSolver* S, size_t l, const double* f, double** out, double* final_out, double final_scale,
                               const PlStokesOp* sop, const double* rs, double* z) {
    MgLevel* L = S->levels[l];
    MgLevel* C = S->levels[l + 1];
    const PlGeom& g = L->gh.d;
    int npre, npost;
    level_nu(S, l, npre, npost);
    MgTileArgs a{};
    a.op = L->op; a.opc = C->op;
    a.f = rs ? (const double*)L->f : f; a.fout = L->f; a.v = L->v[0]; a.fc = C->f;
    const int TS = (long long)g.lnz * g.lnx >= S->tile32_min_nodes ? 32 : MGT_TS;
    const int own_z = g.lnz - (g.gi0 + g.lnz == g.nz ? 1 : 0), own_x = g.lnx - (g.gj0 + g.lnx == g.nx ? 1 : 0);
    a.tiles_x = (own_x + TS - 1) / TS;
    const dim3 grid((unsigned)(a.tiles_x * ((own_z + TS - 1) / TS)));
    cheb_coeffs(L->lmax, S->cheb_ratio, npre, a.c1, a.c2);
    if (rs) { a.sop = *sop; a.rs = rs; a.z = z; }
#define MGT_PRE(NS, L0) do { if (TS == 32) hipLaunchKernelGGL((k_mg_pre<NS, L0, 32>), grid, dim3(mgt_nt(mgt_pre_nn(NS, 32))), 0, ctx->stream, a); \
                             else hipLaunchKernelGGL((k_mg_pre<NS, L0, MGT_TS>), grid, dim3(mgt_nt(mgt_pre_nn(NS, MGT_TS))), 0, ctx->stream, a); } while (0)
#define MGT_PRE_X(NS) do { if (TS == 32) hipLaunchKernelGGL((k_mg_pre<NS, false, 32, 1>), grid, dim3(mgt_nt(mgt_pre_nn(NS + 1, 32))), 0, ctx->stream, a); \
                           else hipLaunchKernelGGL((k_mg_pre<NS, false, MGT_TS, 1>), grid, dim3(mgt_nt(mgt_pre_nn(NS + 1, MGT_TS))), 0, ctx->stream, a); } while (0)
    if (L->dist) {
        (void)pl_halo(ctx, g, (double*)a.f, 2, g.plane, npre + 2);
        if (npre == 1) MGT_PRE_X(1); else if (npre == 2) MGT_PRE_X(2); else MGT_PRE_X(3);
        if (!C->dist) (void)pl_gather_blocks(ctx, C->gh.d, C->f, 2, C->gh.d.plane);
    }
    else if (rs) { if (npre == 1) MGT_PRE(1, true); else if (npre == 2) MGT_PRE(2, true); else MGT_PRE(3, true); }
    else { if (npre == 1) MGT_PRE(1, false); else if (npre == 2) MGT_PRE(2, false); else MGT_PRE(3, false); }
#undef MGT_PRE
#undef MGT_PRE_X
    double* ec = nullptr;
    bool wf = false;
    vcycle<double>(ctx, S, l + 1, C->f, &ec, &wf, nullptr, 1.0, 0, nullptr);
    if (L->dist && C->dist) (void)pl_halo(ctx, C->gh.d, ec, 2, C->gh.d.plane, 4);
    a.ec = ec; a.out = final_out ? final_out : L->v[2]; a.oscale = final_out ? final_scale : 1.0; a.out_plane = g.plane;
    cheb_coeffs(L->lmax, S->cheb_ratio, npost, a.c1, a.c2);
#define MGT_POST(NS) do { if (TS == 32) hipLaunchKernelGGL((k_mg_post<NS, 32>), grid, dim3(mgt_nt(mgt_post_nn(NS, 32))), 0, ctx->stream, a); \
                          else hipLaunchKernelGGL((k_mg_post<NS, MGT_TS>), grid, dim3(mgt_nt(mgt_post_nn(NS, MGT_TS))), 0, ctx->stream, a); } while (0)
    if (npost == 1) MGT_POST(1); else if (npost == 2) MGT_POST(2); else MGT_POST(3);
#undef MGT_POST
    *out = final_out ? nullptr : L->v[2];
}

template <typename T>
__global__ __launch_bounds__(256) void k_copy_vel(PlGeom g, const T* __restrict__ e, double* __restrict__ z, double oscale) {
    PL_NODE_PROLOGUE(g)
    (void)i; (void)j;
    z[c] = (double)e[c] * oscale; z[c + g.plane] = (double)e[c + g.plane] * oscale;
}

__global__ __launch_bounds__(256) void k_vv_close_frame(PlVvOp op, double* __restrict__ z) {
    const PlGeom& g = op.g;
    const int t = blockIdx.x * 256 + threadIdx.x;
    int i, j;
    if (t < 3 * g.lnx) { const int q = t / g.lnx; i = q == 0 ? 0 : g.nz - 3 + q; j = g.gj0 + t % g.lnx; }
    else if (t < 3 * g.lnx + 3 * g.lnz) { const int u = t - 3 * g.lnx, q = u / g.lnz; j = q == 0 ? 0 : g.nx - 3 + q; i = g.gi0 + u % g.lnz; }
    else return;
    const int li = i - g.gi0, lj = j - g.gj0;
    if (li < 0 || li >= g.lnz || lj < 0 || lj >= g.lnx) return;
    const long long c = pl_idx(g, li, lj), P = g.plane;
    int moff; double s;
    int cls = vv_cls_z(op, i, j, moff, s);
    if (cls == VV_ZERO) z[c] = 0.0; else if (cls == VV_SLAVE) z[c] = s * z[c + moff];
    cls = vv_cls_x(op, i, j, moff, s);
    if (cls == VV_ZERO) z[c + P] = 0.0; else if (cls == VV_SLAVE) z[c + P] = s * z[c + moff + P];
}

template <typename T>
static int stokes_precond_t(pl_ctx* ctx, PlSolver* S, const double* rs, double* z) {
    PlStokesOp op = ctx->sop;
    MgLevel* L0 = S->levels[0];
    MgLevel* L = L0;
    const PlGeom& g = ctx->sop.g;
    const bool f32 = std::is_same<T, float>::value;
    const double kappa = f32 ? S->kappa : 1.0, fscale = f32 ? S->kappa / S->sigma : 1.0, oscale = f32 ? 1.0 / S->kappa : 1.0;
    int e_last = 0, f_depth = 0;
    const bool deep = level_deep_plan(S, L0, 0, e_last, f_depth);
    ExtViewT<T> V = ext_view<T>(ctx, L0, deep ? f_depth : 0);
    if (L0->dist) {
        if (deep) PL_TRY(pl_halo(ctx, g, (double*)rs, 3, g.plane, f_depth + 1));
        else PL_TRY(pl_halo(ctx, g, (double*)rs + 2 * g.plane, 1, g.plane));
    }
    op.g = V.op.g; op.etas -= V.sh; op.etan -= V.sh; if (op.rho) op.rho -= V.sh;
    op.iKc /= S->schur_scale;
    if constexpr (std::is_same<T, double>::value) {
        if (mg_fused_level_ok(ctx, S, 0)) {
            double* e2 = nullptr;
            vcycle_fused_level(ctx, S, 0, nullptr, &e2, z, 1.0, &op, rs, z);
            PL_HIP(ctx, hipGetLastError());
            S->nprec++;
            return 0;
        }
    }
    int npre0, npost0;
    level_nu(S, 0, npre0, npost0);
    if constexpr (std::is_same<T, double>::value) {
        const double hmean = 0.5 * ((ctx->geom.zc.back() - ctx->geom.zc.front()) / (ctx->nz - 1) + (ctx->geom.xc.back() - ctx->geom.xc.front()) / (ctx->nx - 1));
        const double sig = ctx->sop.Kc / hmean, ik = 1.0 / S->kappa;
        const bool range_ok = std::isfinite(sig) && sig > 0.0 && ik * std::min(1.0, sig) > 1e-30 && ik * std::max(1.0, sig) < 1e22;
        if (S->l0_mixed && S->l0_mixed_now && !S->any_line && range_ok && !L0->dist && !L0->op.szz && g_vv_vec && (g.plane % 2) == 0 && S->levels.size() > 1 && npre0 == 1 && npost0 == 1 &&
            S->fuse_first && ctx->nranks == 1 && !S->levels[1]->dist && !S->levels[1]->f32) {
            MgLevel* C = S->levels[1];
            for (float** q : {&L0->ff, &L0->rf, &L0->vf[0]}) if (!*q) PL_TRY(fmalloc0(ctx, q, (size_t)2 * g.plane * sizeof(float)));
            float* ff = L0->ff; float* rf = L0->rf; float* v1f = L0->vf[0];
            double* vd = L0->v[0];
            PlVvOpT<float> cls{};
            cls.g = L0->op.g; cls.slave_x = L0->op.slave_x; cls.slave_z0 = L0->op.slave_z0; cls.slave_zL = L0->op.slave_zL;
            cls.s0 = (float)L0->op.s0; cls.sL = (float)L0->op.sL;
            const double lmax = L0->lmax, lmin = lmax / S->cheb_ratio, c2 = 1.0 / (0.5 * (lmax + lmin));
            const dim3 rows2 = pl_grid_rows2(g), bl(64, 4);
            hipLaunchKernelGGL(k_prec_stage1_v2<float>, rows2, bl, 0, ctx->stream, op, cls, rs, z, ff, v1f, c2, 1.0, 1.0);
            hipLaunchKernelGGL((k_vv_first2<double, float, float>), dim3(3 * rows2.x + 3 * rows2.y + 2), bl, 0, ctx->stream, L0->op, (const float*)ff, v1f, c2, 2,
                               ctx->sop.anchor_i, ctx->sop.anchor_j, ctx->sop.wall_ps);
            hipLaunchKernelGGL((k_vv_sweep2<1, double, float, float, float>), rows2, bl, 0, ctx->stream, L0->op, (const float*)v1f, (const float*)nullptr,
                               (const float*)ff, rf, 0.0, 0.0, 1.0f);
            hipLaunchKernelGGL((k_vv_restrict<float, double>), grid2d(C->gh.d), bl, 0, ctx->stream, g, C->op, (const float*)rf, C->f, 1.0);
            double* ec = nullptr; bool wf = false;
            vcycle<double>(ctx, S, 1, C->f, &ec, &wf, nullptr, 1.0, 0, nullptr);
            hipLaunchKernelGGL((k_vv_prolong_add<double, double, float>), grid2d(g), bl, 0, ctx->stream, L0->op, C->gh.d, (const double*)ec, (const float*)v1f, vd);
            hipLaunchKernelGGL((k_vv_sweep2<0, double, double, double, float>), rows2, bl, 0, ctx->stream, L0->op, (const double*)vd, (const double*)nullptr,
                               (const float*)ff, z, 0.0, c2, 1.0);
            PL_HIP(ctx, hipGetLastError());
            S->nprec++;
            return 0;
// ... 1261 lines not shown
    const bool fuse = !multi && !(getenv("PYLAMP_HEAT_FUSE") && atoi(getenv("PYLAMP_HEAT_FUSE")) == 0);
    auto read_norms = [&]() {
        xmass = hs[HC_PQ]; rho_g = hs[HC_RAD];
        cheb_ok = cheb_env != 0 && rho_g > 0.0 && rho_g < 0.97 && std::isfinite(rho_g);
    };
    if (multi) { PL_TRY(fetch()); read_norms(); }
    if (unsuited) *unsuited = false;
    if (multi && !cheb_ok) {
        if (unsuited) *unsuited = true;
        double ms0 = 0; PL_TRY(pl_timer_stop_ms(ctx, &ms0));
        return 0;
    }
    st->iterations = 0; st->converged = 0; st->rel_residual = 0.0; st->error_estimate = 0.0;
    S->napply = 0;
    double ref = 0.0, hist[4] = {0, 0, 0, 0};
    int it = 0;
    if (multi && E > 0) PL_TRY(pl_halo(ctx, g, (double*)b_dev, 1, g.plane, E));
    for (int pass = 0; pass < 5; pass++) {
        if (multi && E > 0) {
            PL_TRY(pl_halo(ctx, g, x, 1, g.plane, E));
            PL_HIP(ctx, hipMemsetAsync(d, 0, pb, ctx->stream));
        }
        hipLaunchKernelGGL(k_heat_cg_residual, grX, bl, 0, ctx->stream, X.op, b_dev - X.sh, (const double*)(x - X.sh), r - X.sh, dinv - X.sh, z - X.sh, pa - X.sh,
                           d - X.sh, 0, S->hc_part, own);
        hipLaunchKernelGGL(k_heat_cg_scalars, dim3(1), dim3(1024), 0, ctx->stream, nb, (const double*)S->hc_part, sc, 0);
        if (multi) {
            PL_HIP(ctx, hipMemcpyAsync(sc + HC_ALPHA, sc + HC_REF, sizeof(double), hipMemcpyDeviceToDevice, ctx->stream));
            PL_TRY(pl_comm_allreduce_dev(ctx, sc + HC_RZ, 3, 0));
            PL_HIP(ctx, hipMemcpyAsync(sc + HC_REF, sc + HC_ALPHA, sizeof(double), hipMemcpyDeviceToDevice, ctx->stream));
        }
        S->napply++;
        PL_TRY(fetch());
        if (pass == 0 && !multi) read_norms();
        if (pass == 0) ref = std::sqrt(hs[HC_REF]);
        double znorm = std::sqrt(hs[HC_ZZ]);
        if (!(ref > 0.0)) { st->converged = 1; break; }
        st->rel_residual = znorm / ref;
        if (znorm <= rtol * ref || it >= maxit || pass == 4) { st->converged = znorm <= rtol * ref ? 1 : 0; break; }
        double* pold = pa; double* pnew = pbuf;
        bool first = true, ok = true;
        if (cheb_ok) {
            const double sigma = 1.0 / rho_g, target = 0.25 * rtol * ref / znorm;
            int ks = 1; double t0 = 1.0, t1 = sigma;
            while (1.0 / t1 > target && ks < 200) { const double t2 = 2.0 * sigma * t1 - t0; t0 = t1; t1 = t2; ks++; }
            ks = std::min(ks, std::max(maxit - it, 1));
            const double theta = 1.0, delta = rho_g;
            double rho_old = 1.0 / sigma;
            double* bufs[4] = {d, pa, pbuf, S->hc[8]};
            int ext = E - 1;
            auto coef = [&](int k, double* c1, double* c2) {
                if (k == 0) { *c1 = 0.0; *c2 = 1.0 / theta; }
                else { const double rr = 1.0 / (2.0 * sigma - rho_old); *c1 = rr * rho_old; *c2 = 2.0 * rr / delta; rho_old = rr; }
            };
            for (int k = 0; k < ks;) {
                const int kf = fuse ? std::min(ks - k, PL_HEAT_KMAX) : 1;
                if (kf >= 2) {
                    HeatChebCoef cf{};
                    for (int q = 0; q < kf; q++) coef(k + q, &cf.c1[q], &cf.c2[q]);
                    launch_heat_cheb_fused(ctx, kf, hop, bufs[0], bufs[1], r, bufs[2], bufs[3], cf);
                    S->heat_fused_launches++;
                    std::swap(bufs[0], bufs[2]); std::swap(bufs[1], bufs[3]);
                    k += kf; S->napply += kf;
                    continue;
                }
                double c1, c2;
                coef(k, &c1, &c2);
                if (multi && ext < 0) {
                    PL_TRY(pl_halo(ctx, g, S->hc3, 3, g.plane, E));
                    ext = E - 1;
                }
                const HeatExt V = heat_ext(ctx, hop, multi ? ext : 0);
                hipLaunchKernelGGL(k_heat_cheb, grid2d(V.op.g), bl, 0, ctx->stream, V.op, (const double*)(bufs[0] - V.sh), (const double*)(bufs[1] - V.sh),
                                   (const double*)(r - V.sh), (const double*)(dinv - V.sh), bufs[2] - V.sh, c1, c2);
                double* nx = bufs[2]; bufs[2] = bufs[1]; bufs[1] = bufs[0]; bufs[0] = nx;
                ext--;
                k++; S->napply++;
            }
            it += ks;
            hipLaunchKernelGGL(k_add_inplace, grid1d(g.plane), dim3(256), 0, ctx->stream, (long long)g.plane, x, (const double*)bufs[0]);
            close_walls(x);
            continue;
        }
        while (it < maxit) {
            it++;
            hipLaunchKernelGGL(k_heat_cg_apply, gr, bl, 0, ctx->stream, hop, (const double*)z, (const double*)pold, pnew, q, (const double*)sc, first ? 0 : 1, S->hc_part);
            hipLaunchKernelGGL(k_heat_cg_scalars, dim3(1), dim3(1024), 0, ctx->stream, nb, (const double*)S->hc_part, sc, 1);
            hipLaunchKernelGGL(k_heat_cg_update, gr, bl, 0, ctx->stream, g, (const double*)pnew, (const double*)q, (const double*)dinv, d, r, z, (const double*)sc, S->hc_part);
            hipLaunchKernelGGL(k_heat_cg_scalars, dim3(1), dim3(1024), 0, ctx->stream, nb, (const double*)S->hc_part, sc, 2);
            S->napply++;
            std::swap(pold, pnew); first = false;
            if (it + 3 < S->hc_last_its && it < maxit) continue;
            PL_TRY(fetch());
            hist[it & 3] = hs[HC_HS];
            znorm = std::sqrt(hs[HC_ZZ]);
            if (!std::isfinite(znorm) || !(hs[HC_PQ] > 0.0)) { ok = false; break; }
            if (znorm <= rtol * ref) break;
        }
        hipLaunchKernelGGL(k_add_inplace, grid1d(g.plane), dim3(256), 0, ctx->stream, (long long)g.plane, x, (const double*)d);
        close_walls(x);
        if (!ok) break;
    }
    PL_HIP(ctx, hipGetLastError());
    st->iterations = it;
    S->hc_last_its = st->converged ? it : 0;
    if (xmass > 0.0) st->error_estimate = std::sqrt(std::fabs(hist[0]) + std::fabs(hist[1]) + std::fabs(hist[2]) + std::fabs(hist[3])) / std::sqrt(xmass);
    if (cheb_ok && xmass > 0.0 && hs[HC_RZ] >= 0.0) st->error_estimate = std::sqrt(hs[HC_RZ] / (1.0 - rho_g)) / std::sqrt(xmass);
    double ms = 0;
    PL_TRY(pl_timer_stop_ms(ctx, &ms));
    st->solve_ms = ms; st->operator_applies = S->napply; st->precond_applies = 0;
    *x_out = x;
    return 0;
}

int pl_heat_solve_device(pl_ctx* ctx, const double* b_dev, double rtol, int maxit, pl_solve_stats* st,
                         double** x_out, const double* x0_dev) {
    PlSolver* S = solver_of(ctx);
    if (ctx->nz >= 3 && ctx->nx >= 3 && (ctx->nranks == 1 || std::min(ctx->geom.d.lnz, ctx->geom.d.lnx) >= 2)) {
        bool unsuited = false;
        PL_TRY(heat_solve_cg(ctx, S, b_dev, rtol, maxit, st, x_out, x0_dev, &unsuited));
        if (!unsuited) return 0;
    }
    const PlGeom& g = ctx->geom.d;
    size_t pb = (size_t)g.plane * sizeof(double);
    for (int k = 0; k < 11; k++) if (!S->h[k]) PL_TRY(dmalloc0(ctx, &S->h[k], pb));
    PL_TRY(scal_alloc(ctx, S));
    PL_TRY(pl_timer_start(ctx));
    PlHeatOp hop = ctx->hop;
    S->napply = 0;
    VecOp A = [&](const double* in, double* out) -> int {
        PL_TRY(pl_halo(ctx, g, (double*)in, 1, g.plane));
        pl_launch_heat_apply(ctx, hop, in, out, true);
        S->napply++;
        return 0;
    };
    double* b = S->h[8];
    PL_HIP(ctx, hipMemcpyAsync(b, b_dev, pb, hipMemcpyDeviceToDevice, ctx->stream));
    hipLaunchKernelGGL(k_heat_dinv, grid2d(g), dim3(64, 4), 0, ctx->stream, hop, b);
    BicgVecs w{S->h[0], S->h[1], S->h[2], S->h[3], S->h[4], S->h[5], nullptr, nullptr, S->h[6], S->h[9], S->h[10]};
    if (x0_dev) PL_HIP(ctx, hipMemcpyAsync(S->h[7], x0_dev, pb, hipMemcpyDeviceToDevice, ctx->stream));
    PL_TRY(bicgstab(ctx, S, g, 1, A, nullptr, b, S->h[7], x0_dev != nullptr, rtol, maxit, w, st));
    double ms = 0;
    PL_TRY(pl_timer_stop_ms(ctx, &ms));
    st->solve_ms = ms; st->operator_applies = S->napply; st->precond_applies = 0;
    *x_out = S->h[7];
    return 0;
}

extern "C" int pl_heat_fused_launches(pl_ctx* ctx, long long* n) {
    if (!n) return pl_fail(ctx, "pl_heat_fused_launches: n is NULL");
    *n = solver_of(ctx)->heat_fused_launches;
    return 0;
}

extern "C" int pl_heat_solve(pl_ctx* ctx, const double* rhs, double* x, double rtol, int maxit,
                             pl_solve_stats* stats) {
    if (!ctx->hop_ready) return pl_fail(ctx, "heat operator not set");
    if (!x) return pl_fail(ctx, "pl_heat_solve: x is NULL");
    PL_HIP(ctx, hipSetDevice(ctx->device));
    const PlGeom& g = ctx->geom.d;
    double* db;
    PL_TRY(pl_buf(ctx, "api_hx", (size_t)g.plane * sizeof(double), &db));
    if (rhs) PL_TRY(pl_plane_upload(ctx, g, rhs, db));
    else pl_launch_heat_rhs(ctx, ctx->hop, ctx->bufs["f_T"], ctx->bufs["H"], db);
    pl_solve_stats st{};
    if (rtol <= 0) rtol = 1e-12;
    if (maxit <= 0) maxit = 2000;
    double* xs = nullptr;
    PL_TRY(pl_heat_solve_device(ctx, db, rtol, maxit, &st, &xs));
    PL_TRY(pl_plane_download(ctx, g, xs, x));
    if (stats) *stats = st;
    return 0;
}
```

pylamp_amd/pylamp_stokes.py:

```python
import ctypes as C

import numpy as np

from .pylamp_const import *
from .pylamp_const import DIM, IZ, IX
from . import _lib
from ._context import get_context

BC_TYPE_NOSLIP = 0
BC_TYPE_FREESLIP = 1
BC_TYPE_CYCLIC = 2
BC_TYPE_FLOWTHRU = 4

DEFAULT_RTOL = 1e-7
DEFAULT_MAXIT = 400


def gidx(idxs, nx, dim):
    if len(idxs) != dim:
        raise Exception("num of idxs != dimensions")
    if dim == 2:
        ret = idxs[IZ] * nx[IX] * (dim + 1) + idxs[IX] * (dim + 1)
    else:
        print("!!! NOT IMPLEMENTED")
        raise Exception("gidx: only 2D is implemented")
    return ret


def x2vp(x, nx):
    dof = int(np.prod(nx)) * (DIM + 1)
    x = np.asarray(x)
    newvel = [[]] * DIM
    for d in range(DIM):
        newvel[d] = x[d:dof:DIM + 1].reshape(nx)
    newpres = x[DIM:dof:DIM + 1].reshape(nx)
    return (newvel, newpres)


class StokesOperator:

    def __init__(self, ctx, nx, coeffs):
        self._ctx = ctx
        self.nx = [int(nx[0]), int(nx[1])]
        n = 3 * self.nx[0] * self.nx[1]
        self.shape = (n, n)
        self.dtype = np.dtype(np.float64)
        self.last_stats = None
        self._coeffs = coeffs
        self._gen = -1
        self._activate()
        kc = C.c_double(); kb = C.c_double()
        ctx.check(ctx.lib.pl_stokes_get_scaling(ctx.handle(), C.byref(kc), C.byref(kb)))
        self.Kcont, self.Kbond = kc.value, kb.value
        ctx.operators.add(self)

    def _activate(self):
        ctx = self._ctx
        if self._gen == ctx.stokes_gen and self._gen >= 0:
            return
        es, en, rho, bc, surfstab, tstep, theta = self._coeffs
        bc_arr = (C.c_int * 4)(*bc)
        ctx.check(ctx.lib.pl_stokes_set_coeffs(ctx.handle(), _lib.dptr(es), _lib.dptr(en), _lib.dptr(rho), bc_arr,
                                               surfstab, tstep, theta))
        ctx.stokes_gen += 1
        self._gen = ctx.stokes_gen

    def matvec(self, x):
        x = _lib.f64(x).reshape(-1)
        if x.size != self.shape[0]:
            raise Exception("dimension mismatch")
        self._activate()
        y = np.empty_like(x)
        self._ctx.check(self._ctx.lib.pl_stokes_apply(self._ctx.handle(), _lib.dptr(x), _lib.dptr(y)))
        return y

    dot = matvec

    def __matmul__(self, x):
        return self.matvec(x)

    def rhs(self):
        self._activate()
        r = np.empty(self.shape[0])
        self._ctx.check(self._ctx.lib.pl_stokes_rhs(self._ctx.handle(), _lib.dptr(r)))
        return r

    def residual_dd(self, rhs, x):
        rhs = _lib.f64(rhs).reshape(-1); x = _lib.f64(x).reshape(-1)
        if x.size != self.shape[0] or rhs.size != self.shape[0]:
            raise Exception("dimension mismatch")
        self._activate()
        r = np.empty_like(x)
        self._ctx.check(self._ctx.lib.pl_stokes_residual_dd(self._ctx.handle(), _lib.dptr(rhs), _lib.dptr(x), _lib.dptr(r)))
        return r

    def direct_info(self):
        band = C.c_int(); nb = C.c_int(); fms = C.c_double(); sms = C.c_double(); ns = C.c_int()
        self._ctx.check(self._ctx.lib.pl_stokes_direct_info(self._ctx.handle(), C.byref(band), C.byref(nb), C.byref(fms), C.byref(sms),
                                                            C.byref(ns)))
        return {"band": band.value, "nb": nb.value, "factor_ms": fms.value, "solve_ms": sms.value, "nsolve": ns.value}

    def precond(self, r):
        r = _lib.f64(r).reshape(-1)
        z = np.empty_like(r)
        self._activate()
        self._ctx.check(self._ctx.lib.pl_stokes_precond_apply(self._ctx.handle(), _lib.dptr(r), _lib.dptr(z)))
        return z

    def mg_info(self):
        n = C.c_int(); lm = (C.c_double * 32)()
        self._ctx.check(self._ctx.lib.pl_stokes_mg_info(self._ctx.handle(), C.byref(n), lm, 32))
        return n.value, [lm[k] for k in range(n.value)]

    def mg_plan(self):
        n = self.mg_info()[0]
        sm = (C.c_int * 32)(); nu = (C.c_int * 4)(); ratio = C.c_double(); wall = C.c_int()
        self._ctx.check(self._ctx.lib.pl_stokes_mg_plan(self._ctx.handle(), sm, 32, nu, C.byref(ratio), C.byref(wall)))
        return dict(smoother=[sm[k] for k in range(n)], nu=(nu[0], nu[1]), nu0=(nu[2], nu[3]), ratio=ratio.value, wall=bool(wall.value))

    def mg_precision(self):
        n = C.c_int(); nf = C.c_int()
        self._ctx.check(self._ctx.lib.pl_stokes_mg_precision(self._ctx.handle(), C.byref(n), C.byref(nf)))
        return n.value, nf.value

    def set_mg_precision(self, fp32, min_nodes=0):
        self._ctx.check(self._ctx.lib.pl_stokes_set_mg_precision(self._ctx.handle(), int(bool(fp32)), int(min_nodes)))

    def tocsc(self):
        import scipy.sparse as sp
        nz, nxx = self.nx
        ii, jj = np.meshgrid(np.arange(nz), np.arange(nxx), indexing='ij')
        rows, cols, vals = [], [], []
        node = (ii * nxx + jj)
        for ci in range(3):
            for cj in range(3):
                mask = ((ii % 3) == ci) & ((jj % 3) == cj)
                for q in range(3):
                    e = np.zeros((nz, nxx, 3))
                    e[mask, q] = 1.0
                    y = self.matvec(e.reshape(-1)).reshape(nz, nxx, 3)
                    ri, rj, rq = np.nonzero(y)
                    pi = ri + ((ci - ri % 3 + 1) % 3 - 1)
                    pj = rj + ((cj - rj % 3 + 1) % 3 - 1)
                    ok = (pi >= 0) & (pi < nz) & (pj >= 0) & (pj < nxx)
                    rows.append((node[ri, rj] * 3 + rq)[ok])
                    cols.append((pi * nxx + pj)[ok] * 3 + q)
                    vals.append(y[ri, rj, rq][ok])
        A = sp.coo_matrix((np.concatenate(vals), (np.concatenate(rows), np.concatenate(cols))), shape=self.shape)
        return A.tocsc()


def makeStokesMatrix(nx, grid, f_etas, f_etan, f_rho, bc, surfstab=False, tstep=None, surfstab_theta=0.5,
                     strict_reference=True):
    ctx = get_context(nx, grid)
    if surfstab and tstep is None:
        raise Exception("surface stabilization needs predetermined tstep")
    es, en, rho = (np.array(a, dtype=np.float64, order="C") for a in (f_etas, f_etan, f_rho))
    for a in (es, en, rho):
        if a.shape != (int(nx[0]), int(nx[1])):
            raise Exception("field shape does not match nx")
    coeffs = (es, en, rho, [int(b) for b in bc], 1 if surfstab else 0, float(tstep) if tstep is not None else 0.0,
              float(surfstab_theta) if strict_reference else -float(surfstab_theta))
    A = StokesOperator(ctx, nx, coeffs)
    return (A, A.rhs())


def solve(A, rhs, x0=None, rtol=DEFAULT_RTOL, maxit=DEFAULT_MAXIT):
    ctx = A._ctx
    A._activate()
    rhs = _lib.f64(rhs).reshape(-1)
    x = np.zeros_like(rhs) if x0 is None else _lib.f64(x0).reshape(-1).copy()
    st = _lib.SolveStats()
    ctx.check(ctx.lib.pl_stokes_solve(ctx.handle(), _lib.dptr(rhs), _lib.dptr(x), 0 if x0 is None else 1, float(rtol),
                                      int(maxit), C.byref(st)))
    A.last_stats = st.as_dict()
    return x
```

Before: 194.6 million.

## Rewrite LDS multigrid tail kernel with per-thread cached row coefficients

Restructures the single-block coarse-level multigrid tail kernel so that each thread owns one finest-level node and one coarse-level node, keeping stencil coefficients, classification and the right-hand side in registers rather than recomputing them from shared tables every sweep. Chebyshev coefficients are precomputed into shared memory and broadcast through readfirstlane, and the three-buffer rotation becomes a two-buffer ping-pong with a smaller LDS pool. The fit checks are tightened so the new kernel only runs on small grids, and launch counters are added for diagnostics. In exchange the kernel uses more registers per thread and applies to fewer configurations, which then fall back to the global-memory tail kernel.

```diff
diff --git a/include/pylamp_hip.h b/include/pylamp_hip.h
--- a/include/pylamp_hip.h
+++ b/include/pylamp_hip.h
@@ -85,6 +85,7 @@
 int  pl_stokes_sweep_bench(pl_ctx* ctx, int reps, double* avg_ms);
 int  pl_stokes_mg_precision(pl_ctx* ctx, int* nlevels, int* nlevels_fp32);
 int  pl_stokes_set_mg_precision(pl_ctx* ctx, int fp32, long long min_nodes);
+int  pl_mg_tail_launches(pl_ctx* ctx, long long* lds, long long* global);
 
 int  pl_heat_set_coeffs(pl_ctx* ctx, const double* zmp, const double* xmp, const double* T,
                         const double* kz, const double* kx, const double* cp, const double* rho,
diff --git a/pylamp_amd/_lib.py b/pylamp_amd/_lib.py
--- a/pylamp_amd/_lib.py
+++ b/pylamp_amd/_lib.py
@@ -157,6 +157,7 @@
     "pl_stokes_mg_precision": (C.c_int, [C.c_void_p, c_int_p, c_int_p]),
     "pl_stokes_set_mg_precision": (C.c_int, [C.c_void_p, C.c_int, C.c_longlong]),
     "pl_stokes_sweep_bench": (C.c_int, [C.c_void_p, C.c_int, c_double_p]),
+    "pl_mg_tail_launches": (C.c_int, [C.c_void_p, C.POINTER(C.c_longlong), C.POINTER(C.c_longlong)]),
     "pl_heat_set_coeffs": (C.c_int, [C.c_void_p] + [c_double_p] * 8 + [c_int_p, c_double_p, C.c_double]),
     "pl_heat_apply": (C.c_int, [C.c_void_p, c_double_p, c_double_p]),
     "pl_heat_rhs": (C.c_int, [C.c_void_p, c_double_p]),
diff --git a/pylamp_amd/csrc/pl_solver.hip b/pylamp_amd/csrc/pl_solver.hip
--- a/pylamp_amd/csrc/pl_solver.hip
+++ b/pylamp_amd/csrc/pl_solver.hip
@@ -1384,6 +1384,7 @@
     double* hc[9] = {nullptr}; double* hc_part = nullptr; int hc_nb = 0, hc_last_its = 0;
     int napply = 0, nprec = 0;
     long long heat_fused_launches = 0;
+    long long tail_lds_launches = 0, tail_global_launches = 0;
 };
 
 static PlSolver* solver_of(pl_ctx* ctx) {
@@ -1984,6 +1985,7 @@
                                          double final_scale, int f_valid_depth, const int* first_done_anchor);
 static bool mg_fused_level_ok(pl_ctx* ctx, const PlSolver* S, size_t l);
 static bool mg_tail_lds_fits(const PlSolver* S, size_t l);
+static bool mg_tail_cheb_fits(int nlev, int nu_pre, int nu_post, int coarse_sweeps);
 __global__ void k_mg_tail_lds(TailArgs a);
 static void vcycle_fused_level(pl_ctx* ctx, PlSolver* S, size_t l, const double* f, double** out, double* final_out, double final_scale,
                                const PlStokesOp* sop, const double* rs, double* z);
@@ -2037,10 +2039,14 @@
                 ta.L[q].op = T_->op; ta.L[q].f = T_->f; ta.L[q].r = T_->r; ta.L[q].lmax = T_->lmax;
                 for (int b = 0; b < 3; b++) ta.L[q].v[b] = T_->v[b];
             }
-            if (S->fused && !L->dist && !L->op.szz && ta.nu_pre >= 1 && ta.nu_post >= 1 && ta.coarse_sweeps >= 1 && mg_tail_lds_fits(S, l))
+            if (S->fused && !L->dist && !L->op.szz && ta.nu_pre >= 1 && ta.nu_post >= 1 && ta.coarse_sweeps >= 1 && mg_tail_lds_fits(S, l) &&
+                mg_tail_cheb_fits(ta.nlev, ta.nu_pre, ta.nu_post, ta.coarse_sweeps)) {
                 hipLaunchKernelGGL(k_mg_tail_lds, dim3(1), dim3(1024), 0, ctx->stream, ta);
-            else
+                S->tail_lds_launches++;
+            } else {
                 hipLaunchKernelGGL(k_mg_tail, dim3(1), dim3(1024), 0, ctx->stream, ta);
+                S->tail_global_launches++;
+            }
             *out = L->v[0];
             return;
         }
@@ -2134,75 +2140,6 @@
     if (i == op.g.nz - 2 && op.slave_zL) { da = -1; s = op.sL; return VV_SLAVE; }
     return VV_INT;
 }
-template <bool NEED_A>
-__device__ inline void mgt_row_z(const MgtTab& t, const int CR, const double* vz, const double* vx, int c, int a, int b, double& Av, double& dg) {
-    const double rdz_i = t.rdz[a + 1], rdz_m = t.rdz[a], rDz_i = t.rDz[a + 1];
-    const double rdx_j = t.rdx[b + 1], rDx_j = t.rDx[b + 1], rDx_p = t.rDx[b + 2];
-    const double esC = t.es[c], esE = t.es[c + 1];
-    const double cN = 4.0 * t.en[c] * rdz_i * rDz_i, cS = 4.0 * t.en[c - CR] * rdz_m * rDz_i;
-    const double cE = 2.0 * esE * rDx_p * rdx_j, cW = 2.0 * esC * rDx_j * rdx_j;
-    dg = cN + cS + cE + cW;
-    if (NEED_A) {
-        const double xE = 2.0 * esE * rDz_i * rdx_j, xW = 2.0 * esC * rDz_i * rdx_j;
-        const double v0 = vz[c];
-        Av = cN * (vz[c + CR] - v0) - cS * (v0 - vz[c - CR]) + cE * (vz[c + 1] - v0) - cW * (v0 - vz[c - 1]) +
-             xE * (vx[c + 1] - vx[c - CR + 1]) - xW * (vx[c] - vx[c - CR]);
-    }
-}
-template <bool NEED_A>
-__device__ inline void mgt_row_x(const MgtTab& t, const int CR, const double* vz, const double* vx, int c, int a, int b, double& Av, double& dg) {
-    const double rdx_j = t.rdx[b + 1], rdx_m = t.rdx[b], rDx_j = t.rDx[b + 1];
-    const double rdz_i = t.rdz[a + 1], rDz_i = t.rDz[a + 1], rDz_p = t.rDz[a + 2];
-    const double esC = t.es[c], esN = t.es[c + CR];
-    const double cE = 4.0 * t.en[c] * rdx_j * rDx_j, cW = 4.0 * t.en[c - 1] * rdx_m * rDx_j;
-    const double cN = 2.0 * esN * rDz_p * rdz_i, cS = 2.0 * esC * rDz_i * rdz_i;
-    dg = cE + cW + cN + cS;
-    if (NEED_A) {
-        const double zN = 2.0 * esN * rDx_j * rdz_i, zS = 2.0 * esC * rDx_j * rdz_i;
-        const double v0 = vx[c];
-        Av = cE * (vx[c + 1] - v0) - cW * (v0 - vx[c - 1]) + cN * (vx[c + CR] - v0) - cS * (v0 - vx[c - CR]) +
-             zN * (vz[c + CR] - vz[c + CR - 1]) - zS * (vz[c] - vz[c - 1]);
-    }
-}
-
-struct MgtTile {
-    int ci0, cj0;
-    int CR, NR;
-    MgtTab t;
-    __device__ inline void first(const PlVvOp& op, const double* fz, const double* fx, double* oz, double* ox, double c2, int a, int b) const {
-        const int i = ci0 + a, j = cj0 + b, c = a * CR + b;
-        int d; double s, Av, dg;
-        double o = 0.0;
-        int cls = mgt_cls_z(op, i, j, d, s);
-        if (cls != VV_ZERO && b + d >= 1 && b + d <= CR - 2) { mgt_row_z<false>(t, CR, nullptr, nullptr, c + d, a, b + d, Av, dg); o = (-s * c2 * fz[c + d]) * pl_rcp(dg); }
-        oz[c] = o;
-        o = 0.0;
-        cls = mgt_cls_x(op, i, j, d, s);
-        if (cls != VV_ZERO && a + d >= 1 && a + d <= NR - 2) { mgt_row_x<false>(t, CR, nullptr, nullptr, c + d * CR, a + d, b, Av, dg); o = (-s * c2 * fx[c + d * CR]) * pl_rcp(dg); }
-        ox[c] = o;
-    }
-    __device__ inline void cheb(const PlVvOp& op, const double* vz, const double* vx, const double* pz, const double* px, const double* fz,
-                                const double* fx, double c1, double c2, int a, int b, double& oz, double& ox) const {
-        const int i = ci0 + a, j = cj0 + b, c = a * CR + b;
-        int d; double s, Av, dg;
-        oz = 0.0; ox = 0.0;
-        int cls = mgt_cls_z(op, i, j, d, s);
-        if (cls != VV_ZERO && b + d >= 1 && b + d <= CR - 2) {
-            const int cm = c + d;
-            mgt_row_z<true>(t, CR, vz, vx, cm, a, b + d, Av, dg);
-            const double v0 = vz[cm], mom = (c1 != 0.0) ? c1 * (v0 - (pz ? pz[cm] : 0.0)) : 0.0;
-            oz = s * (v0 + mom + (c2 * (Av - fz[cm])) * pl_rcp(dg));
-        }
-        cls = mgt_cls_x(op, i, j, d, s);
-        if (cls != VV_ZERO && a + d >= 1 && a + d <= NR - 2) {
-            const int cm = c + d * CR;
-            mgt_row_x<true>(t, CR, vz, vx, cm, a + d, b, Av, dg);
-            const double v0 = vx[cm], mom = (c1 != 0.0) ? c1 * (v0 - (px ? px[cm] : 0.0)) : 0.0;
-            ox = s * (v0 + mom + (c2 * (Av - fx[cm])) * pl_rcp(dg));
-        }
-    }
-};
-
 __device__ inline void mgt_load_table(double* dst, const double* tab, int first_global, int count, int n) {
     for (int k = threadIdx.x; k < count; k += blockDim.x) {
         const int gk = first_global + k;
@@ -2520,175 +2457,287 @@
 }
 
 #define MGT_TAIL_POOL 18600
+#define MGT_TAIL_CHEB 256
+#define MGT_TAIL_LDS 11520
 struct TailLvl { int base, NR, CR, N; };
 #define TL_V(D, buf, c) (pool + (D).base + (2 * (buf) + (c)) * (D).N)
-#define TL_F(D, c) (pool + (D).base + (6 + (c)) * (D).N)
-#define TL_ES(D) (pool + (D).base + 8 * (D).N)
-#define TL_EN(D) (pool + (D).base + 9 * (D).N)
-#define TL_TAB(D, k) (pool + (D).base + 10 * (D).N + ((k) < 2 ? (k) * ((D).NR + 3) : 2 * ((D).NR + 3) + ((k) - 2) * ((D).CR + 3)))
-#define TL_FOR_NODES(g)                                                                                                     \
-    for (int idx = threadIdx.x, nxm_ = (g).nx - 1, pw_ = (nxm_ & (nxm_ - 1)) == 0, sh_ = 31 - __clz(nxm_), i, j;            \
-         idx < ((g).nz - 1) * nxm_ && (i = pw_ ? idx >> sh_ : idx / nxm_, j = idx - i * nxm_, true); idx += MGT_NT)
-__device__ inline MgtTile mgt_tail_tile(double* pool, const TailLvl& D) {
-    MgtTile T; T.ci0 = -1; T.cj0 = -1; T.CR = D.CR; T.NR = D.NR;
-    T.t.es = TL_ES(D); T.t.en = TL_EN(D); T.t.rdz = TL_TAB(D, 0); T.t.rDz = TL_TAB(D, 1); T.t.rdx = TL_TAB(D, 2); T.t.rDx = TL_TAB(D, 3);
-    return T;
-}
-__device__ inline void mgt_tail_smooth(double* pool, const TailLevel& L, const TailLvl& D, int& cur, int& prv, int& nxt, int nsweep, double ratio, bool zero_guess) {
-    const double lmax = L.lmax, lmin = lmax / ratio;
+#define TL_ES(D) (pool + (D).base + 4 * (D).N)
+#define TL_EN(D) (pool + (D).base + 5 * (D).N)
+#define TL_TAB(D, k) (pool + (D).base + 6 * (D).N + ((k) < 2 ? (k) * ((D).NR + 3) : 2 * ((D).NR + 3) + ((k) - 2) * ((D).CR + 3)))
+__host__ __device__ inline TailLvl mgt_tail_lvl(const PlGeom& g, int base) {
+    TailLvl D; D.base = base; D.NR = g.nz + 2; D.CR = g.nx + 2; D.N = D.NR * D.CR;
+    return D;
+}
+__host__ __device__ inline int mgt_tail_lvl_size(const TailLvl& D) { return 6 * D.N + 2 * (D.NR + 3) + 2 * (D.CR + 3); }
+struct MgtTailRows {
+    MgtC kz, kx; int ij, o;
+    __device__ inline int i() const { return ij >> 16; }
+    __device__ inline int j() const { return ij & 0xffff; }
+};
+__device__ inline int mgt_tail_dz(const MgtTailRows& R) { return R.kz.cm - R.o; }
+__device__ inline int mgt_tail_dx(const MgtTailRows& R) { const int t = R.kx.cm - R.o; return (t > 0) - (t < 0); }
+__device__ inline double mgt_uniform(double x) {
+    const long long b = __double_as_longlong(x);
+    const unsigned lo = __builtin_amdgcn_readfirstlane((unsigned)b), hi = __builtin_amdgcn_readfirstlane((unsigned)(b >> 32));
+    return __longlong_as_double((long long)(((unsigned long long)hi << 32) | lo));
+}
+__device__ inline void mgt_tail_rows(MgtTailRows& R, const PlVvOp& op, const TailLvl& D, int q) {
+    const int nxm = op.g.nx - 1;
+    const int i = q / nxm, j = q - i * nxm;
+    R.ij = i << 16 | j; R.o = (i + 1) * D.CR + (j + 1);
+    R.kz = mgt_classify<true>(op, D.CR, D.NR, -1, -1, i + 1, j + 1);
+    R.kx = mgt_classify<false>(op, D.CR, D.NR, -1, -1, i + 1, j + 1);
+    const double s0 = op.s0, sL = op.sL;
+    R.kx.s = R.kx.d > 0 ? s0 : (R.kx.d < 0 ? sL : 1.0);
+}
+__device__ inline void mgt_tail_coefficients(double* pool, const TailLvl& D, MgtTailRows& R) {
+    MgtTab t; t.es = TL_ES(D); t.en = TL_EN(D); t.rdz = TL_TAB(D, 0); t.rDz = TL_TAB(D, 1); t.rdx = TL_TAB(D, 2); t.rDx = TL_TAB(D, 3);
+    mgt_coefficients<true>(R.kz, t, D.CR); mgt_coefficients<false>(R.kx, t, D.CR);
+}
+__device__ inline void mgt_tail_cheb_coeffs(double* ch, double lmax, double ratio, int n) {
+    const double lmin = lmax / ratio;
     const double theta = 0.5 * (lmax + lmin), delta = 0.5 * (lmax - lmin), sigma = theta / delta;
     double rho_old = 1.0 / sigma;
-    const MgtTile T = mgt_tail_tile(pool, D);
-    for (int k = 0; k < nsweep; k++) {
+    for (int k = 0; k < n; k++) {
         double c1, c2;
         if (k == 0) { c1 = 0.0; c2 = 1.0 / theta; }
         else { const double rho = 1.0 / (2.0 * sigma - rho_old); c1 = rho * rho_old; c2 = 2.0 * rho / delta; rho_old = rho; }
-        double* const nz_ = TL_V(D, nxt, 0); double* const nx_ = TL_V(D, nxt, 1);
-        const double* const cz = TL_V(D, cur, 0); const double* const cx = TL_V(D, cur, 1);
-        const bool noprev = k == 1 && zero_guess;
-        const double* const pz = noprev ? nullptr : TL_V(D, prv, 0); const double* const px = noprev ? nullptr : TL_V(D, prv, 1);
-        TL_FOR_NODES(L.op.g) {
-            const int ra = i + 1, rb = j + 1;
-            if (k == 0 && zero_guess) T.first(L.op, TL_F(D, 0), TL_F(D, 1), nz_, nx_, c2, ra, rb);
-            else {
-                double oz, ox;
-                T.cheb(L.op, cz, cx, pz, px, TL_F(D, 0), TL_F(D, 1), c1, c2, ra, rb, oz, ox);
-                nz_[ra * D.CR + rb] = oz; nx_[ra * D.CR + rb] = ox;
-            }
-        }
+        ch[2 * k] = c1; ch[2 * k + 1] = c2;
+    }
+}
+__device__ inline void mgt_tail_smooth(double* pool, const double* ch, const TailLvl& D, MgtTailRows& R, bool mine, int& cur, int nsweep, bool zero_guess) {
+    double pvz = 0.0, pvx = 0.0;
+    double c1 = mgt_uniform(ch[0]), c2 = mgt_uniform(ch[1]);
+    for (int k = 0; k < nsweep; k++) {
+        if (mine) {
+            double oz, ox;
+            if (k == 0 && zero_guess) {
+                oz = R.kz.on ? (-R.kz.s * c2 * R.kz.f) * R.kz.rdg : 0.0;
+                ox = R.kx.on ? (-R.kx.s * c2 * R.kx.f) * R.kx.rdg : 0.0;
+            } else {
+                mgt_cheb(R.kz, R.kx, D.CR, TL_V(D, cur, 0), TL_V(D, cur, 1), pvz, pvx, c1, c2, oz, ox);
+            }
+            TL_V(D, cur ^ 1, 0)[R.o] = oz; TL_V(D, cur ^ 1, 1)[R.o] = ox;
+        }
+        double n1 = 0.0, n2 = 0.0;
+        if (k + 1 < nsweep) { n1 = ch[2 * k + 2]; n2 = ch[2 * k + 3]; }
         __syncthreads();
-        const int o = prv; prv = cur; cur = nxt; nxt = o;
-    }
+        c1 = mgt_uniform(n1); c2 = mgt_uniform(n2);
+        cur ^= 1;
+    }
+}
+__device__ inline void mgt_tail_residual(double* pool, const TailLvl& D, const MgtTailRows& R, bool mine, int cur) {
+    if (mine) {
+        double v0, rz = 0.0, rx = 0.0;
+        if (R.kz.interior) rz = R.kz.f - mgt_av_z(R.kz, D.CR, TL_V(D, cur, 0), TL_V(D, cur, 1), v0);
+        if (R.kx.interior) rx = R.kx.f - mgt_av_x(R.kx, D.CR, TL_V(D, cur, 0), TL_V(D, cur, 1), v0);
+        TL_V(D, cur ^ 1, 0)[R.o] = rz; TL_V(D, cur ^ 1, 1)[R.o] = rx;
+    }
+    __syncthreads();
+}
+__device__ inline void mgt_tail_prolong(double* pool, const TailLvl& D, const TailLvl& Dc, const PlGeom& gc, const MgtTailRows& R, bool mine, int cur,
+                                        int curc) {
+    if (mine) {
+        const double* const ez = TL_V(Dc, curc, 0); const double* const ex = TL_V(Dc, curc, 1);
+        double oz = 0.0, ox = 0.0;
+        if (R.kz.on) {
+            const int i = R.i(), jm = R.j() + mgt_tail_dz(R), I0 = i >> 1, I1 = (i + 1) >> 1;
+            int Jn = jm >> 1, Jo = (jm & 1) ? Jn + 1 : Jn - 1;
+            Jn = min(max(Jn, 0), gc.nx - 2); Jo = min(max(Jo, 0), gc.nx - 2);
+            const double pa = 0.5 * (ez[(I0 + 1) * Dc.CR + Jn + 1] + ez[(I1 + 1) * Dc.CR + Jn + 1]);
+            const double pb = 0.5 * (ez[(I0 + 1) * Dc.CR + Jo + 1] + ez[(I1 + 1) * Dc.CR + Jo + 1]);
+            oz = R.kz.s * (TL_V(D, cur, 0)[R.kz.cm] + (0.75 * pa + 0.25 * pb));
+        }
+        if (R.kx.on) {
+            const int im = R.i() + mgt_tail_dx(R), j = R.j(), J0 = j >> 1, J1 = (j + 1) >> 1;
+            int In = im >> 1, Io = (im & 1) ? In + 1 : In - 1;
+            In = min(max(In, 0), gc.nz - 2); Io = min(max(Io, 0), gc.nz - 2);
+            const double pa = 0.5 * (ex[(In + 1) * Dc.CR + J0 + 1] + ex[(In + 1) * Dc.CR + J1 + 1]);
+            const double pb = 0.5 * (ex[(Io + 1) * Dc.CR + J0 + 1] + ex[(Io + 1) * Dc.CR + J1 + 1]);
+            ox = R.kx.s * (TL_V(D, cur, 1)[R.kx.cm] + (0.75 * pa + 0.25 * pb));
+        }
+        TL_V(D, cur ^ 1, 0)[R.o] = oz; TL_V(D, cur ^ 1, 1)[R.o] = ox;
+    }
+    __syncthreads();
 }
 __global__ __launch_bounds__(MGT_NT) void k_mg_tail_lds(TailArgs a) {
-    __shared__ double pool[MGT_TAIL_POOL];
-    __shared__ TailLvl lv[PL_TAIL_MAX_LEVELS];
-    __shared__ int rot[PL_TAIL_MAX_LEVELS];
+    __shared__ double pool[MGT_TAIL_LDS];
+    __shared__ double chb[2 * MGT_TAIL_CHEB];
     const int tid = threadIdx.x;
-    for (int k = tid; k < MGT_TAIL_POOL; k += MGT_NT) pool[k] = 0.0;
-    if (tid == 0) {
-        int q = 0;
-        for (int l = 0; l < a.nlev; l++) {
+    const int nlev = a.nlev, ksm = max(a.nu_pre, a.nu_post);
+    const TailLevel& L0 = a.L[0]; const PlGeom& g0 = L0.op.g; const TailLvl D0 = mgt_tail_lvl(g0, 0);
+    MgtTailRows A, B = {};
+    B.kz.s = 1.0;
+    const bool haveA = tid < (g0.nz - 1) * (g0.nx - 1);
+    mgt_tail_rows(A, L0.op, D0, haveA ? tid : 0);
+    if (haveA) {
+        const long long c = pl_idx(g0, A.i() - g0.gi0, A.j() - g0.gj0);
+        if (A.kz.on) A.kz.f = L0.f[c + A.kz.d];
+        if (A.kx.on) A.kx.f = L0.f[c + (long long)A.kx.d * g0.pitch + g0.plane];
+    }
+    double e0[2][2]; int e0o[2];
+#pragma unroll
+    for (int q = 0; q < 2; q++) {
+        const int idx = tid + q * MGT_NT;
+        const bool ok = idx < g0.nz * g0.nx;
+        const int i = ok ? idx / g0.nx : 0, j = ok ? idx - i * g0.nx : 0;
+        const long long c = pl_idx(g0, i - g0.gi0, j - g0.gj0);
+        e0[q][0] = L0.op.etas[c]; e0[q][1] = L0.op.etan[c];
+        e0o[q] = ok ? (i + 1) * D0.CR + (j + 1) : -1;
+    }
+    int lb = 0, eco = -1, ecN = 0;
+    bool riz = false, rix = false;
+    const double* pes = nullptr; const double* pen = nullptr;
+    {
+        int base = mgt_tail_lvl_size(D0), start = 0, vstart = 0;
+        for (int l = 1; l < nlev; l++) {
+            const PlVvOp& op = a.L[l].op; const PlGeom& g = op.g; const TailLvl D = mgt_tail_lvl(g, base);
+            const int n = (g.nz - 1) * (g.nx - 1), nv = g.nz * g.nx;
+            if (tid >= start && tid < start + n) {
+                lb = l;
+                mgt_tail_rows(B, op, D, tid - start);
+                int d; double s;
+                riz = B.kz.on && mgt_cls_z(op, B.i(), B.j() + B.kz.d, d, s) == VV_INT;
+                rix = B.kx.on && mgt_cls_x(op, B.i() + B.kx.d, B.j(), d, s) == VV_INT;
+            }
+            if (tid >= vstart && tid < vstart + nv) {
+                const int q = tid - vstart, i = q / g.nx, j = q - i * g.nx;
+                const long long c = pl_idx(g, i - g.gi0, j - g.gj0);
+                pes = op.etas + c; pen = op.etan + c;
+                eco = D.base + 4 * D.N + (i + 1) * D.CR + (j + 1); ecN = D.N;
+            }
+            start = (start + n + 63) & ~63; vstart += nv; base += mgt_tail_lvl_size(D);
+        }
+    }
+    int tdst = -1;
+    const double* ptab = nullptr;
+    {
+        int base = 0, tstart = 0;
+        for (int l = 0; l < nlev; l++) {
+            const PlVvOp& op = a.L[l].op; const TailLvl D = mgt_tail_lvl(op.g, base);
+#pragma unroll
+            for (int k = 0; k < 4; k++) {
+                const double* const tab = k == 0 ? op.rdz : k == 1 ? op.rDz : k == 2 ? op.rdx : op.rDx;
+                const int n = k < 2 ? op.g.nz : op.g.nx, count = n + 5, e = tid - tstart;
+                if (e >= 0 && e < count) { tdst = (int)(TL_TAB(D, k) - pool) + e; ptab = e < n + 2 * PL_TOFF ? tab + e : nullptr; }
+                tstart += count;
+            }
+            base += mgt_tail_lvl_size(D);
+        }
+    }
+    const double ec0 = pes ? *pes : 0.0, ec1 = pen ? *pen : 0.0, tabv = ptab ? *ptab : 0.0;
+    {
+        const int l = __builtin_amdgcn_readfirstlane(tid >> 6);
+        if (l < nlev && (tid & 63) == 0) {
             const PlGeom& g = a.L[l].op.g;
-            TailLvl D; D.base = q; D.NR = g.nz + 2; D.CR = g.nx + 2; D.N = D.NR * D.CR;
-            q += 10 * D.N + 2 * (D.NR + 3) + 2 * (D.CR + 3);
-            lv[l] = D;
-        }
-    }
+            double ratio = 0.4 * g.nz * g.nx; if (ratio < 30.0) ratio = 30.0;
+            if (l == nlev - 1) mgt_tail_cheb_coeffs(chb + 2 * l * ksm, a.L[l].lmax, ratio, a.coarse_sweeps);
+            else mgt_tail_cheb_coeffs(chb + 2 * l * ksm, a.L[l].lmax, a.ratio, ksm);
+        }
+    }
+    {
+        int base = 0;
+        for (int l = 0; l < nlev; l++) {
+            const TailLvl D = mgt_tail_lvl(a.L[l].op.g, base);
+            for (int k = tid; k < 4 * D.N; k += MGT_NT) pool[base + k] = 0.0;
+            base += mgt_tail_lvl_size(D);
+        }
+    }
+#pragma unroll
+    for (int q = 0; q < 2; q++)
+        if (e0o[q] >= 0) { TL_ES(D0)[e0o[q]] = e0[q][0]; TL_EN(D0)[e0o[q]] = e0[q][1]; }
+    if (eco >= 0) { pool[eco] = ec0; pool[eco + ecN] = ec1; }
+    if (tdst >= 0) pool[tdst] = tabv;
     __syncthreads();
-    for (int l = 0; l < a.nlev; l++) {
-        const TailLevel& L = a.L[l]; const PlGeom& g = L.op.g; const TailLvl D = lv[l];
-        for (int idx = tid; idx < g.nz * g.nx; idx += MGT_NT) {
-            const int i = idx / g.nx, j = idx - i * g.nx;
-            const long long c = pl_idx(g, i - g.gi0, j - g.gj0);
-            const int o = (i + 1) * D.CR + (j + 1);
-            TL_ES(D)[o] = L.op.etas[c]; TL_EN(D)[o] = L.op.etan[c];
-            if (l == 0) { TL_F(D, 0)[o] = L.f[c]; TL_F(D, 1)[o] = L.f[c + g.plane]; }
-        }
-        mgt_load_table(TL_TAB(D, 0), L.op.rdz, -2, D.NR + 3, g.nz); mgt_load_table(TL_TAB(D, 1), L.op.rDz, -2, D.NR + 3, g.nz);
-        mgt_load_table(TL_TAB(D, 2), L.op.rdx, -2, D.CR + 3, g.nx); mgt_load_table(TL_TAB(D, 3), L.op.rDx, -2, D.CR + 3, g.nx);
-    }
-    __syncthreads();
-    for (int l = 0; l < a.nlev; l++) {
-        const TailLevel& L = a.L[l]; const PlGeom& g = L.op.g; const TailLvl D = lv[l];
-        int cur = 0, prv = 1, nxt = 2;
-        if (l == a.nlev - 1) {
-            double ratio = 0.4 * g.nz * g.nx; if (ratio < 30.0) ratio = 30.0;
-            mgt_tail_smooth(pool, L, D, cur, prv, nxt, a.coarse_sweeps, ratio, true);
-            if (tid == 0) rot[l] = cur | (prv << 2) | (nxt << 4);
-            break;
-        }
-        mgt_tail_smooth(pool, L, D, cur, prv, nxt, a.nu_pre, a.ratio, true);
-        if (tid == 0) rot[l] = cur | (prv << 2) | (nxt << 4);
-        const MgtTile T = mgt_tail_tile(pool, D);
-        double* const rz = TL_V(D, nxt, 0); double* const rx = TL_V(D, nxt, 1);
-        const double* const cz = TL_V(D, cur, 0); const double* const cx = TL_V(D, cur, 1);
-        TL_FOR_NODES(g) {
-            const int ra = i + 1, rb = j + 1, o = ra * D.CR + rb;
-            int d; double s, Av, dg, vz = 0.0, vx = 0.0;
-            if (mgt_cls_z(L.op, i, j, d, s) == VV_INT) { mgt_row_z<true>(T.t, D.CR, cz, cx, o, ra, rb, Av, dg); vz = TL_F(D, 0)[o] - Av; }
-            if (mgt_cls_x(L.op, i, j, d, s) == VV_INT) { mgt_row_x<true>(T.t, D.CR, cz, cx, o, ra, rb, Av, dg); vx = TL_F(D, 1)[o] - Av; }
-            rz[o] = vz; rx[o] = vx;
-        }
-        __syncthreads();
-        const TailLevel& Cn = a.L[l + 1]; const TailLvl Dc = lv[l + 1];
-        double* const fz = TL_F(Dc, 0); double* const fx = TL_F(Dc, 1);
-        TL_FOR_NODES(Cn.op.g) {
-            const int b0 = (2 * i + 1) * D.CR + (2 * j + 1);
-            int d; double s, oz = 0.0, ox = 0.0;
-            if (vv_cls_z(Cn.op, i, j, d, s) == VV_INT) {
-                const double wz[3] = {0.25, 0.5, 0.25}, wx[4] = {0.125, 0.375, 0.375, 0.125};
-#pragma unroll
-                for (int u = 0; u < 3; u++)
-#pragma unroll
-                    for (int w = 0; w < 4; w++) oz += wz[u] * wx[w] * rz[b0 + (u - 1) * D.CR + (w - 1)];
-            }
-            if (vv_cls_x(Cn.op, i, j, d, s) == VV_INT) {
-                const double wz[4] = {0.125, 0.375, 0.375, 0.125}, wx[3] = {0.25, 0.5, 0.25};
-#pragma unroll
-                for (int u = 0; u < 4; u++)
-#pragma unroll
-                    for (int w = 0; w < 3; w++) ox += wz[u] * wx[w] * rx[b0 + (u - 1) * D.CR + (w - 1)];
-            }
-            const int oc = (i + 1) * Dc.CR + (j + 1);
-            fz[oc] = oz; fx[oc] = ox;
-        }
-        __syncthreads();
-    }
-    __syncthreads();
-    for (int l = a.nlev - 2; l >= 0; l--) {
-        const TailLevel& L = a.L[l]; const PlGeom& g = L.op.g; const TailLvl D = lv[l];
-        const PlGeom& gc = a.L[l + 1].op.g; const TailLvl Dc = lv[l + 1];
-        int cur = rot[l] & 3, prv = (rot[l] >> 2) & 3, nxt = (rot[l] >> 4) & 3;
-        const int curc = rot[l + 1] & 3;
-        const double* const ez = TL_V(Dc, curc, 0); const double* const ex = TL_V(Dc, curc, 1);
-        const double* const cz = TL_V(D, cur, 0); const double* const cx = TL_V(D, cur, 1);
-        double* const wz_ = TL_V(D, nxt, 0); double* const wx_ = TL_V(D, nxt, 1);
-        TL_FOR_NODES(g) {
-            const int o = (i + 1) * D.CR + (j + 1);
-            int d; double s, oz = 0.0, ox = 0.0;
-            if (mgt_cls_z(L.op, i, j, d, s) != VV_ZERO) {
-                const int jm = j + d, I0 = i >> 1, I1 = (i + 1) >> 1;
-                int Jn = jm >> 1, Jo = (jm & 1) ? Jn + 1 : Jn - 1;
-                Jn = min(max(Jn, 0), gc.nx - 2); Jo = min(max(Jo, 0), gc.nx - 2);
-                const double pa = 0.5 * (ez[(I0 + 1) * Dc.CR + Jn + 1] + ez[(I1 + 1) * Dc.CR + Jn + 1]);
-                const double pb = 0.5 * (ez[(I0 + 1) * Dc.CR + Jo + 1] + ez[(I1 + 1) * Dc.CR + Jo + 1]);
-                oz = s * (cz[o + d] + (0.75 * pa + 0.25 * pb));
-            }
-            if (mgt_cls_x(L.op, i, j, d, s) != VV_ZERO) {
-                const int im = i + d, J0 = j >> 1, J1 = (j + 1) >> 1;
-                int In = im >> 1, Io = (im & 1) ? In + 1 : In - 1;
-                In = min(max(In, 0), gc.nz - 2); Io = min(max(Io, 0), gc.nz - 2);
-                const double pa = 0.5 * (ex[(In + 1) * Dc.CR + J0 + 1] + ex[(In + 1) * Dc.CR + J1 + 1]);
-                const double pb = 0.5 * (ex[(Io + 1) * Dc.CR + J0 + 1] + ex[(Io + 1) * Dc.CR + J1 + 1]);
-                ox = s * (cx[o + d * D.CR] + (0.75 * pa + 0.25 * pb));
-            }
-            wz_[o] = oz; wx_[o] = ox;
-        }
-        __syncthreads();
-        { const int o = cur; cur = nxt; nxt = o; }
-        mgt_tail_smooth(pool, L, D, cur, prv, nxt, a.nu_post, a.ratio, false);
-        if (tid == 0) rot[l] = cur | (prv << 2) | (nxt << 4);
-        __syncthreads();
+    if (haveA) mgt_tail_coefficients(pool, D0, A);
+    int base = mgt_tail_lvl_size(D0);
+    for (int l = 1; l < nlev; l++) {
+        const TailLvl D = mgt_tail_lvl(a.L[l].op.g, base);
+        if (lb == l) mgt_tail_coefficients(pool, D, B);
+        base += mgt_tail_lvl_size(D);
+    }
+    const int cur_pre = a.nu_pre & 1, cur_coarse = a.coarse_sweeps & 1, cur_post = (a.nu_pre + 1 + a.nu_post) & 1;
+    int cur = 0;
+    if (nlev == 1) {
+        mgt_tail_smooth(pool, chb, D0, A, haveA, cur, a.coarse_sweeps, true);
+    } else {
+        TailLvl D = D0;
+        for (int l = 0; l < nlev; l++) {
+            const bool coarsest = l == nlev - 1, mine = l == 0 ? haveA : lb == l;
+            const double* const ch = chb + 2 * l * ksm;
+            cur = 0;
+            if (l == 0) {
+                mgt_tail_smooth(pool, ch, D, A, mine, cur, a.nu_pre, true);
+                mgt_tail_residual(pool, D, A, mine, cur);
+            } else {
+                mgt_tail_smooth(pool, ch, D, B, mine, cur, coarsest ? a.coarse_sweeps : a.nu_pre, true);
+                if (coarsest) break;
+                mgt_tail_residual(pool, D, B, mine, cur);
+            }
+            if (lb == l + 1) {
+                const double* const rz = TL_V(D, cur ^ 1, 0); const double* const rx = TL_V(D, cur ^ 1, 1);
+                const int rbz = (2 * B.i() + 1) * D.CR + 2 * (B.j() + mgt_tail_dz(B)) + 1;
+                const int rbx = (2 * (B.i() + mgt_tail_dx(B)) + 1) * D.CR + 2 * B.j() + 1;
+                double oz = 0.0, ox = 0.0;
+                if (riz) {
+                    const double wz[3] = {0.25, 0.5, 0.25}, wx[4] = {0.125, 0.375, 0.375, 0.125};
+#pragma unroll
+                    for (int u = 0; u < 3; u++)
+#pragma unroll
+                        for (int w = 0; w < 4; w++) oz += wz[u] * wx[w] * rz[rbz + (u - 1) * D.CR + (w - 1)];
+                }
+                if (rix) {
+                    const double wz[4] = {0.125, 0.375, 0.375, 0.125}, wx[3] = {0.25, 0.5, 0.25};
+#pragma unroll
+                    for (int u = 0; u < 4; u++)
+#pragma unroll
+                        for (int w = 0; w < 3; w++) ox += wz[u] * wx[w] * rx[rbx + (u - 1) * D.CR + (w - 1)];
+                }
+                B.kz.f = oz; B.kx.f = ox;
+            }
+            __syncthreads();
+            D = mgt_tail_lvl(a.L[l + 1].op.g, D.base + mgt_tail_lvl_size(D));
+        }
+        for (int l = nlev - 2; l >= 0; l--) {
+            const TailLvl Dc = D;
+            D = mgt_tail_lvl(a.L[l].op.g, 0); D.base = Dc.base - mgt_tail_lvl_size(D);
+            const double* const ch = chb + 2 * l * ksm;
+            const int curc = l + 1 == nlev - 1 ? cur_coarse : cur_post;
+            cur = cur_pre;
+            if (l == 0) {
+                mgt_tail_prolong(pool, D, Dc, a.L[l + 1].op.g, A, haveA, cur, curc);
+                cur ^= 1;
+                mgt_tail_smooth(pool, ch, D, A, haveA, cur, a.nu_post, false);
+            } else {
+                mgt_tail_prolong(pool, D, Dc, a.L[l + 1].op.g, B, lb == l, cur, curc);
+                cur ^= 1;
+                mgt_tail_smooth(pool, ch, D, B, lb == l, cur, a.nu_post, false);
+            }
+        }
     }
     {
-        const TailLevel& L = a.L[0]; const PlGeom& g = L.op.g; const TailLvl D = lv[0];
-        const int cur = rot[0] & 3;
-        const double* const cz = TL_V(D, cur, 0); const double* const cx = TL_V(D, cur, 1);
-        for (int idx = tid; idx < g.nz * g.nx; idx += MGT_NT) {
-            const int i = idx / g.nx, j = idx - i * g.nx, o = (i + 1) * D.CR + (j + 1);
-            const long long c = pl_idx(g, i - g.gi0, j - g.gj0);
-            L.v[0][c] = cz[o]; L.v[0][c + g.plane] = cx[o];
-        }
-    }
+        const double* const cz = TL_V(D0, cur, 0); const double* const cx = TL_V(D0, cur, 1);
+        for (int idx = tid; idx < g0.nz * g0.nx; idx += MGT_NT) {
+            const int i = idx / g0.nx, j = idx - i * g0.nx, o = (i + 1) * D0.CR + (j + 1);
+            const long long c = pl_idx(g0, i - g0.gi0, j - g0.gj0);
+            L0.v[0][c] = cz[o]; L0.v[0][c + g0.plane] = cx[o];
+        }
+    }
+}
+static bool mg_tail_cheb_fits(int nlev, int nu_pre, int nu_post, int coarse_sweeps) {
+    return (long long)(nlev - 1) * std::max(nu_pre, nu_post) + coarse_sweeps <= MGT_TAIL_CHEB;
 }
 static bool mg_tail_lds_fits(const PlSolver* S, size_t l) {
-    long long need = 0;
+    long long need = 0, lds = 0, coarse_threads = 0, coarse_nodes = 0, table_entries = 0;
     for (size_t q = l; q < S->levels.size(); q++) {
         const PlGeom& g = S->levels[q]->gh.d;
         need += 10LL * (g.nz + 2) * (g.nx + 2) + 2LL * (g.nz + 5) + 2LL * (g.nx + 5);
-    }
-    return need <= MGT_TAIL_POOL;
+        lds += mgt_tail_lvl_size(mgt_tail_lvl(g, 0)); table_entries += 2LL * (g.nz + 5) + 2LL * (g.nx + 5);
+        if (q > l) { coarse_threads = (coarse_threads + 63) / 64 * 64 + (long long)(g.nz - 1) * (g.nx - 1); coarse_nodes += (long long)g.nz * g.nx; }
+    }
+    const PlGeom& g0 = S->levels[l]->gh.d;
+    return need <= MGT_TAIL_POOL && lds <= MGT_TAIL_LDS && (long long)(g0.nz - 1) * (g0.nx - 1) <= MGT_NT && (long long)g0.nz * g0.nx <= 2 * MGT_NT &&
+           coarse_threads <= MGT_NT && coarse_nodes <= MGT_NT && table_entries <= MGT_NT;
 }
 
 static void cheb_coeffs(double lmax, double ratio, int n, double* c1, double* c2) {
@@ -4256,6 +4305,12 @@
     return 0;
 }
 
+extern "C" int pl_mg_tail_launches(pl_ctx* ctx, long long* lds, long long* global) {
+    if (!lds || !global) return pl_fail(ctx, "pl_mg_tail_launches: lds or global is NULL");
+    *lds = solver_of(ctx)->tail_lds_launches; *global = solver_of(ctx)->tail_global_launches;
+    return 0;
+}
+
 extern "C" int pl_heat_solve(pl_ctx* ctx, const double* rhs, double* x, double rtol, int maxit,
                              pl_solve_stats* stats) {
     if (!ctx->hop_ready) return pl_fail(ctx, "heat operator not set");
diff --git a/pylamp_amd/pylamp_stokes.py b/pylamp_amd/pylamp_stokes.py
--- a/pylamp_amd/pylamp_stokes.py
+++ b/pylamp_amd/pylamp_stokes.py
@@ -112,6 +112,11 @@
         self._ctx.check(self._ctx.lib.pl_stokes_mg_info(self._ctx.handle(), C.byref(n), lm, 32))
         return n.value, [lm[k] for k in range(n.value)]
 
+    def mg_tail_launches(self):
+        lds = C.c_longlong(); glob = C.c_longlong()
+        self._ctx.check(self._ctx.lib.pl_mg_tail_launches(self._ctx.handle(), C.byref(lds), C.byref(glob)))
+        return lds.value, glob.value
+
     def mg_plan(self):
         n = self.mg_info()[0]
         sm = (C.c_int * 32)(); nu = (C.c_int * 4)(); ratio = C.c_double(); wall = C.c_int()
```

Measured after the change: 200.3 million, median of 6. +2.9%, better.
